# PetropoulakisPanagiotis/ICP-Variants

Measured on NVIDIA B200. Metric: icp_registrations_per_s, higher is better.
Workload: dtype f32

## Files before the change

### icp_variants_b200/csrc/clouds.cu

```cuda
#include "context.cuh"
#include <stdlib.h>

static int pick_T(int n, bool source = false) {
    if (!source) {
        int T = 3 * ICP_MAX_BITS_PER_AXIS;
        if (const char* e = getenv("ICP_GPU_TARGET_GRID_BITS")) { const int v = atoi(e); if (v >= 3 && v <= 3 * ICP_MAX_BITS_PER_AXIS) T = v; }
        return T;
    }
    int T = 3;
    while (T < 24 && (1ll << T) < (long long)ICP_SOURCE_CELLS_PER_POINT * (long long)(n > 0 ? n : 1)) ++T;
    if (T > 3 * ICP_MAX_BITS_PER_AXIS) T = 3 * ICP_MAX_BITS_PER_AXIS;
    return T;
}

static int ensure_sort(icp_gpu_ctx* ctx, icp_gpu_ctx::SortBufs& sb, int n, int T) {
    const size_t n1 = (size_t)(n > 0 ? n : 1);
    if (ensure(ctx, sb.keys_a, n1 * 4) || ensure(ctx, sb.keys_b, n1 * 4) || ensure(ctx, sb.idx_a, n1 * 4) || ensure(ctx, sb.idx_b, n1 * 4) ||
        ensure(ctx, sb.hist, icp_radix_hist_words(n, T) * 4) || ensure(ctx, sb.msd, ICP_MSD_WORDS * 4)) return ICP_GPU_E_CUDA;
    return 0;
}

static int upload_cloud(icp_gpu_ctx* ctx, const float* xyz, const float* nrm, const uint8_t* rgba, int64_t n, bool device_ptrs,
                        DeviceBuf& pts, DeviceBuf& nrmb, int kind ) {
    const size_t n1 = (size_t)(n > 0 ? n : 1);
    DeviceBuf& bbox = kind == 0 ? ctx->bbox : ctx->sbbox;
    DeviceBuf& grid = kind == 0 ? ctx->grid : ctx->sgrid;
    icp_gpu_ctx::SortBufs& sb = kind == 0 ? ctx->tsort : ctx->ssort;
    const int T = pick_T((int)n, kind == 1);
    if (kind == 0) ctx->T = T; else ctx->Ts = T;
    if (ensure(ctx, pts, n1 * sizeof(float4)) || ensure(ctx, nrmb, n1 * sizeof(float4)) || ensure(ctx, bbox, 64) || ensure(ctx, grid, sizeof(GridParams)) ||
        ensure_sort(ctx, sb, (int)n, T)) return ICP_GPU_E_CUDA;
    const long long hist_words = (long long)icp_radix_hist_words((int)n, T);
    if (n == 0) {
        CU(icp_launch_pack_cloud(nullptr, nullptr, nullptr, 0, (float4*)pts.p, (float4*)nrmb.p, (unsigned int*)bbox.p, T, (GridParams*)grid.p,
                                 (unsigned int*)sb.hist.p, hist_words, 1, ctx->stream));
        ctx->late_pending[kind] = false;
        return 0;
    }
    const float* dx = xyz; const float* dn = nrm; const uint8_t* dc = rgba;
    if (!device_ptrs) {
        DeviceBuf& stage = kind == 0 ? ctx->stage : ctx->stage2;
        const size_t sizes[] = {(size_t)n * 12, nrm ? (size_t)n * 12 : 0, rgba ? (size_t)n * 4 : 0};
        size_t off[3];
        if (ensure(ctx, stage, pack_segments(sizes, 3, off))) return ICP_GPU_E_CUDA;
        char* st = (char*)stage.p;
        if (ctx->packed_once[kind]) CU(cudaStreamWaitEvent(ctx->copy_stream, ctx->ev_packed[kind], 0));
        CU(cudaMemcpyAsync(st + off[0], xyz, sizes[0], cudaMemcpyHostToDevice, ctx->copy_stream));
        CU(cudaEventRecord(ctx->ev_xyz[kind], ctx->copy_stream));
        dx = (const float*)(st + off[0]);
        if (nrm) { CU(cudaMemcpyAsync(st + off[1], nrm, sizes[1], cudaMemcpyHostToDevice, ctx->copy_stream)); dn = (const float*)(st + off[1]); }
        if (rgba) { CU(cudaMemcpyAsync(st + off[2], rgba, sizes[2], cudaMemcpyHostToDevice, ctx->copy_stream)); dc = (const uint8_t*)(st + off[2]); }
        CU(cudaEventRecord(ctx->ev_copied[kind], ctx->copy_stream));
        CU(cudaStreamWaitEvent(ctx->stream, ctx->ev_xyz[kind], 0));
        ctx->late[kind].nrm = dn; ctx->late[kind].rgba = dc; ctx->late[kind].nrmo = (float4*)nrmb.p; ctx->late[kind].ready = ctx->ev_copied[kind];
    }
    ctx->late_pending[kind] = !device_ptrs;
    CU(icp_launch_pack_cloud(dx, dn, dc, (int)n, (float4*)pts.p, (float4*)nrmb.p, (unsigned int*)bbox.p, T, (GridParams*)grid.p,
                             (unsigned int*)sb.hist.p, hist_words, device_ptrs ? 1 : 0, ctx->stream));
    ctx->stats.n_kernel_launches += 1;
    return 0;
}

static int build_grid(icp_gpu_ctx* ctx) {
    const int n = ctx->n_tgt;
    const size_t n1 = (size_t)(n > 0 ? n : 1);
    if (ensure(ctx, ctx->tgt_pts_sorted, n1 * sizeof(float4)) || ensure(ctx, ctx->tgt_nrm_sorted, n1 * sizeof(float4)) ||
        ensure(ctx, ctx->lv_flags, n1 + 64) || ensure(ctx, ctx->lv_tiles, (n1 / 1024 + 2) * 4) ||
        ensure(ctx, ctx->delta_a, (n1 + 2) * 4) || ensure(ctx, ctx->delta_b, (n1 + 2) * 4) ||
        ensure(ctx, ctx->leaf_start, (n1 + 2) * 4) || ensure(ctx, ctx->leaf_rank, (n1 + 2) * 4) || ensure(ctx, ctx->bvh_desc, sizeof(BvhDesc)) ||
        ensure(ctx, ctx->bvh_box, icp_bvh_max_nodes(n) * 2 * sizeof(float4)) ||
        ensure(ctx, ctx->node_rank, (icp_bvh_max_nodes(n) + ICP_BVH_MAX_LEVELS) * 4) ||
        ensure(ctx, ctx->child_start, (icp_bvh_max_nodes(n) + ICP_BVH_MAX_LEVELS) * 4))
        return ICP_GPU_E_CUDA;
    ctx->adj_capacity = (int)(n1 / 4 + 64);
    ctx->adj1_capacity = (int)(n1 / 32 + 64);
    if (ensure(ctx, ctx->adj, (size_t)ctx->adj_capacity * 32 * 4) || ensure(ctx, ctx->adj_gap, (size_t)ctx->adj_capacity * 32 * 4) ||
        ensure(ctx, ctx->adj_box, (size_t)ctx->adj_capacity * 2 * sizeof(float4)) ||
        ensure(ctx, ctx->adj1, (size_t)ctx->adj1_capacity * 32 * 4) || ensure(ctx, ctx->adj1_box, (size_t)ctx->adj1_capacity * 2 * sizeof(float4)))
        return ICP_GPU_E_CUDA;
    int launches = 0;
    if (join_index(ctx)) return ICP_GPU_E_CUDA;
    CU(cudaEventRecord(ctx->ev[0], ctx->stream));
    CU(icp_launch_cloud_sort((const float4*)ctx->tgt_pts.p, (const float4*)ctx->tgt_nrm.p, n, ctx->T, (const GridParams*)ctx->grid.p,
                             (unsigned int*)ctx->tsort.keys_a.p, (unsigned int*)ctx->tsort.keys_b.p, (unsigned int*)ctx->tsort.idx_a.p,
                             (unsigned int*)ctx->tsort.idx_b.p, (unsigned int*)ctx->tsort.hist.p, (float4*)ctx->tgt_pts_sorted.p,
                             (float4*)ctx->tgt_nrm_sorted.p, (unsigned int*)ctx->tsort.msd.p, &ctx->tsort.keys_sorted, &ctx->tsort.msd_shift,
                             ctx->late_pending[0] ? &ctx->late[0] : nullptr, ctx->stream, &launches));
    if (ctx->late_pending[0]) { CU(cudaEventRecord(ctx->ev_packed[0], ctx->stream)); ctx->packed_once[0] = true; ctx->late_pending[0] = false; }
    cudaStream_t ts = getenv("ICP_GPU_NO_AUX_STREAM") ? ctx->stream : ctx->aux_stream;
    if (ts != ctx->stream) { CU(cudaEventRecord(ctx->ev_fork, ctx->stream)); CU(cudaStreamWaitEvent(ts, ctx->ev_fork, 0)); }
    CU(icp_launch_bvh_build((float4*)ctx->tgt_pts_sorted.p, (float4*)ctx->tgt_nrm_sorted.p, n, ctx->T, ctx->tsort.keys_sorted,
                            (const unsigned int*)ctx->bbox.p + 7, (unsigned char*)ctx->lv_flags.p, (unsigned int*)ctx->lv_tiles.p, (int*)ctx->delta_a.p,
                            (int*)ctx->delta_b.p, (unsigned int*)ctx->leaf_rank.p, (unsigned int*)ctx->leaf_start.p, (unsigned int*)ctx->node_rank.p,
                            (unsigned int*)ctx->child_start.p, (BvhDesc*)ctx->bvh_desc.p, (float4*)ctx->bvh_box.p, ctx->n_sms, ts, &launches));
    const bool bottom_up = !getenv("ICP_GPU_ADJ_FROM_ROOT");
    CU(icp_launch_leaf_adjacency((const BvhDesc*)ctx->bvh_desc.p, (const float4*)ctx->bvh_box.p, (const unsigned int*)ctx->child_start.p,
                                 (unsigned int*)ctx->adj1.p, (float4*)ctx->adj1_box.p, ctx->adj1_capacity, 1, nullptr, nullptr, nullptr, 0, ctx->n_sms, ts, &launches));
    CU(icp_launch_leaf_adjacency((const BvhDesc*)ctx->bvh_desc.p, (const float4*)ctx->bvh_box.p, (const unsigned int*)ctx->child_start.p,
                                 (unsigned int*)ctx->adj.p, (float4*)ctx->adj_box.p, ctx->adj_capacity, 0, (const unsigned int*)ctx->node_rank.p,
                                 bottom_up ? (const unsigned int*)ctx->adj1.p : nullptr, (const float4*)ctx->adj1_box.p, ctx->adj1_capacity, ctx->n_sms, ts, &launches,
                                 (float*)ctx->adj_gap.p));
    CU(cudaEventRecord(ctx->ev[1], ts));
    if (ts != ctx->stream) { CU(cudaEventRecord(ctx->ev_index_ready, ts)); ctx->index_pending = true; }
    ctx->stats.n_kernel_launches += (uint64_t)launches;
    ctx->grid_built = true;
    return 0;
}

static int build_source(icp_gpu_ctx* ctx) {
    const int n = ctx->n_src;
    const size_t n1 = (size_t)(n > 0 ? n : 1);
    if (ensure(ctx, ctx->src_pts, n1 * sizeof(float4)) || ensure(ctx, ctx->src_nrm, n1 * sizeof(float4))) return ICP_GPU_E_CUDA;
    int launches = 0;
    CU(icp_launch_cloud_sort((const float4*)ctx->src_raw_pts.p, (const float4*)ctx->src_raw_nrm.p, n, ctx->Ts, (const GridParams*)ctx->sgrid.p,
                             (unsigned int*)ctx->ssort.keys_a.p, (unsigned int*)ctx->ssort.keys_b.p, (unsigned int*)ctx->ssort.idx_a.p,
                             (unsigned int*)ctx->ssort.idx_b.p, (unsigned int*)ctx->ssort.hist.p, (float4*)ctx->src_pts.p,
                             (float4*)ctx->src_nrm.p, nullptr, &ctx->ssort.keys_sorted, &ctx->ssort.msd_shift,
                             ctx->late_pending[1] ? &ctx->late[1] : nullptr, ctx->stream, &launches));
    if (ctx->late_pending[1]) { CU(cudaEventRecord(ctx->ev_packed[1], ctx->stream)); ctx->packed_once[1] = true; ctx->late_pending[1] = false; }
    ctx->stats.n_kernel_launches += (uint64_t)launches;
    return 0;
}

int set_cloud(icp_gpu_ctx* ctx, bool target, const float* xyz, const float* nrm, const uint8_t* rgba, int64_t n, bool dev) {
    if (n < 0 || n > 0x7fffffff / 4 || (n > 0 && !xyz)) return fail(ctx, ICP_GPU_E_ARG, "bad cloud (n=%lld, xyz=%p)", (long long)n, (const void*)xyz);
    if (int rc = enter(ctx)) return rc;
    if (target) {
        if (join_index(ctx)) return ICP_GPU_E_CUDA;
        if (upload_cloud(ctx, xyz, nrm, rgba, n, dev, ctx->tgt_pts, ctx->tgt_nrm, 0)) return ICP_GPU_E_CUDA;
        ctx->n_tgt = (int)n;
        if (build_grid(ctx)) return ICP_GPU_E_CUDA;
    } else {
        if (upload_cloud(ctx, xyz, nrm, rgba, n, dev, ctx->src_raw_pts, ctx->src_raw_nrm, 1)) return ICP_GPU_E_CUDA;
        ctx->n_src = (int)n;
        ctx->src_finite_valid = false; ctx->src_rank_valid = false;
        const size_t n1 = (size_t)(n > 0 ? n : 1);
        if (ensure(ctx, ctx->match_pos, n1 * 4) || ensure(ctx, ctx->match_w, n1 * 4) || ensure(ctx, ctx->match_idx, n1 * 4) ||
            ensure(ctx, ctx->nn_pos, n1 * 4) || ensure(ctx, ctx->nn_leaf, n1 * 4) || ensure(ctx, ctx->qbuf, n1 * sizeof(float4)) ||
            ensure(ctx, ctx->seedbuf, n1 * sizeof(float4))) return ICP_GPU_E_CUDA;
        ctx->n_reduce_blocks = icp_reduce_blocks((int)n, ctx->n_sms);
        if (ensure(ctx, ctx->partials, (size_t)ctx->n_reduce_blocks * ICP_NRED * sizeof(double))) return ICP_GPU_E_CUDA;
        if (build_source(ctx)) return ICP_GPU_E_CUDA;
    }
    ctx->nn_stale = true;
    if (!dev && n > 0) CU(cudaEventSynchronize(ctx->ev_copied[target ? 0 : 1]));
    return ICP_GPU_OK;
}

int fetch_src_rank(icp_gpu_ctx* ctx) {
    if (ctx->src_rank_valid) return 0;
    const size_t n = (size_t)ctx->n_src;
    std::vector<int> order(n);
    if (n > 0) {
        if (ensure(ctx, ctx->order_dev, n * 4)) return ICP_GPU_E_CUDA;
        CU(icp_launch_extract_order((const float4*)ctx->src_pts.p, (int)n, (int*)ctx->order_dev.p, ctx->stream));
        CU(cudaMemcpyAsync(order.data(), ctx->order_dev.p, n * 4, cudaMemcpyDeviceToHost, ctx->stream));
        CU(cudaStreamSynchronize(ctx->stream));
    }
    ctx->src_rank.assign(n, 0);
    for (size_t p = 0; p < n; ++p) ctx->src_rank[(size_t)order[p]] = (int)p;
    ctx->src_rank_valid = true;
    return 0;
}

int fetch_src_finite(icp_gpu_ctx* ctx) {
    if (ctx->src_finite_valid) return 0;
    const size_t n = (size_t)ctx->n_src;
    std::vector<float4> p(n), m(n);
    CU(cudaMemcpyAsync(p.data(), ctx->src_raw_pts.p, n * sizeof(float4), cudaMemcpyDeviceToHost, ctx->stream));
    CU(cudaMemcpyAsync(m.data(), ctx->src_raw_nrm.p, n * sizeof(float4), cudaMemcpyDeviceToHost, ctx->stream));
    CU(cudaStreamSynchronize(ctx->stream));
    ctx->src_finite.resize(n);
    for (size_t i = 0; i < n; ++i) ctx->src_finite[i] = point_finite(&p[i].x, &m[i].x) ? 1 : 0;
    ctx->src_finite_valid = true;
    return 0;
}

int icp_gpu_set_target(icp_gpu_ctx* ctx, const float* xyz, const float* nrm, const uint8_t* rgba, int64_t n) { return set_cloud(ctx, true, xyz, nrm, rgba, n, false); }
int icp_gpu_set_source(icp_gpu_ctx* ctx, const float* xyz, const float* nrm, const uint8_t* rgba, int64_t n) { return set_cloud(ctx, false, xyz, nrm, rgba, n, false); }
int icp_gpu_set_target_dev(icp_gpu_ctx* ctx, const float* xyz, const float* nrm, const uint8_t* rgba, int64_t n) { return set_cloud(ctx, true, xyz, nrm, rgba, n, true); }
int icp_gpu_set_source_dev(icp_gpu_ctx* ctx, const float* xyz, const float* nrm, const uint8_t* rgba, int64_t n) { return set_cloud(ctx, false, xyz, nrm, rgba, n, true); }

int icp_gpu_cloud_from_depth(icp_gpu_ctx* ctx, const float* depth, const uint8_t* rgbx, const float K[9], const float E[16],
                             uint32_t width, uint32_t height, int keep_original_size, uint32_t downsample, float max_distance, int role,
                             float* xyz_out, float* nrm_out, uint8_t* rgba_out, int64_t* n_out) {
    if (!K) return ICP_GPU_E_ARG;
    if (!depth || width == 0 || height == 0 || downsample == 0 || (long long)width * height > 0x7fffffff / 4)
        return fail(ctx, ICP_GPU_E_ARG, "bad depth map (%p, %ux%u, downsample %u)", (const void*)depth, width, height, downsample);
    if (role < ICP_GPU_CLOUD_TARGET || role > ICP_GPU_CLOUD_ONLY) return fail(ctx, ICP_GPU_E_ARG, "role %d", role);
    if (int rc = enter(ctx)) return rc;
    const long long npx = (long long)width * height;
    DepthArgs a; memset(&a, 0, sizeof(a));
    a.width = width; a.height = height; a.downsample = downsample; a.keep_original_size = keep_original_size ? 1 : 0;
    a.n_candidates = (npx + downsample - 1) / downsample;
    a.fovX = K[0]; a.fovY = K[4]; a.cX = K[6]; a.cY = K[7];
    a.half_max_distance = max_distance / 2.f;
    for (int i = 0; i < 16; ++i) a.Einv[i] = (i % 5 == 0) ? 1.f : 0.f;
    if (E) {
        double m[4][8];
        for (int r = 0; r < 4; ++r) for (int c = 0; c < 4; ++c) { m[r][c] = E[r + 4 * c]; m[r][4 + c] = (r == c) ? 1.0 : 0.0; }
        for (int k = 0; k < 4; ++k) {
            int p = k; for (int i = k + 1; i < 4; ++i) if (fabs(m[i][k]) > fabs(m[p][k])) p = i;
            if (m[p][k] == 0.0) return fail(ctx, ICP_GPU_E_ARG, "singular depth extrinsics");
            if (p != k) for (int j = 0; j < 8; ++j) { const double t = m[k][j]; m[k][j] = m[p][j]; m[p][j] = t; }
            const double d = m[k][k];
            for (int j = 0; j < 8; ++j) m[k][j] /= d;
            for (int i = 0; i < 4; ++i) if (i != k) { const double f = m[i][k]; if (f != 0.0) for (int j = 0; j < 8; ++j) m[i][j] -= f * m[k][j]; }
        }
        for (int r = 0; r < 4; ++r) for (int c = 0; c < 4; ++c) a.Einv[r + 4 * c] = (float)m[r][4 + c];
    }
    const size_t nc = (size_t)a.n_candidates, nb = (nc + 255) / 256;
    const size_t depth_bytes = (size_t)npx * 4, color_bytes = rgbx ? (size_t)npx + 3 : 0;
    const size_t in_sizes[] = {depth_bytes, color_bytes}, sizes[] = {nc * 12, nc * 12, nc * 4, nc * 4, (nb + 2) * 4};
    size_t in_off[2], t[5];
    const size_t in_total = pack_segments(in_sizes, 2, in_off), t_end = pack_segments(sizes, 5, t);
    if (ensure(ctx, ctx->prep_in, in_total) || ensure(ctx, ctx->prep_tmp, t_end) || ensure(ctx, ctx->prep_out, t[3])) return ICP_GPU_E_CUDA;
    char* in = (char*)ctx->prep_in.p; char* tmp = (char*)ctx->prep_tmp.p; char* out = (char*)ctx->prep_out.p;
    CU(cudaMemcpyAsync(in, depth, depth_bytes, cudaMemcpyHostToDevice, ctx->stream));
    if (rgbx) CU(cudaMemcpyAsync(in + in_off[1], rgbx, color_bytes, cudaMemcpyHostToDevice, ctx->stream));
    int launches = 0;
    unsigned int* total = (unsigned int*)(tmp + t[4]) + nb;
    CU(icp_launch_depth_cloud((const float*)in, rgbx ? (const unsigned char*)(in + in_off[1]) : nullptr, a, (float*)tmp, (float*)(tmp + t[1]),
                              (unsigned char*)(tmp + t[2]), (unsigned int*)(tmp + t[3]), (unsigned int*)(tmp + t[4]), total,
                              (float*)out, (float*)(out + t[1]), (unsigned char*)(out + t[2]), ctx->stream, &launches));
    ctx->stats.n_kernel_launches += (uint64_t)launches;
    unsigned int n = 0;
    CU(cudaMemcpyAsync(&n, total, 4, cudaMemcpyDeviceToHost, ctx->stream));
    CU(cudaStreamSynchronize(ctx->stream));
    if (n_out) *n_out = (int64_t)n;
    if (n > 0) {
        if (xyz_out) CU(cudaMemcpyAsync(xyz_out, out, (size_t)n * 12, cudaMemcpyDeviceToHost, ctx->stream));
        if (nrm_out) CU(cudaMemcpyAsync(nrm_out, out + t[1], (size_t)n * 12, cudaMemcpyDeviceToHost, ctx->stream));
        if (rgba_out) CU(cudaMemcpyAsync(rgba_out, out + t[2], (size_t)n * 4, cudaMemcpyDeviceToHost, ctx->stream));
    }
    int rc = ICP_GPU_OK;
    if (role != ICP_GPU_CLOUD_ONLY)
        rc = set_cloud(ctx, role == ICP_GPU_CLOUD_TARGET, (const float*)out, (const float*)(out + t[1]), (const uint8_t*)(out + t[2]), (int64_t)n, true);
    if (xyz_out || nrm_out || rgba_out) CU(cudaStreamSynchronize(ctx->stream));
    return rc;
}

int icp_gpu_target_normals(icp_gpu_ctx* ctx, int32_t k, const float viewpoint[3], float* nrm_out, float* curvature_out) {
    if (k < 3 || k > 8) return fail(ctx, ICP_GPU_E_ARG, "k %d (3..8)", k);
    if (int rc = enter(ctx)) return rc;
    if (!ctx->grid_built) return fail(ctx, ICP_GPU_E_STATE, "no target cloud set");
    const int n = ctx->n_tgt;
    if (n <= 0) return ICP_GPU_OK;
    if (join_index(ctx)) return ICP_GPU_E_CUDA;
    if (ensure(ctx, ctx->nrm_out_dev, (size_t)n * 16 + 256)) return ICP_GPU_E_CUDA;
    NormalArgs a; memset(&a, 0, sizeof(a));
    a.pts = (const float4*)ctx->tgt_pts_sorted.p; a.n = n;
    a.bvh_box = (const float4*)ctx->bvh_box.p; a.bvh = (const BvhDesc*)ctx->bvh_desc.p; a.leaf_start = (const unsigned int*)ctx->leaf_start.p;
    a.leaf_rank = (const unsigned int*)ctx->leaf_rank.p; a.child_start = (const unsigned int*)ctx->child_start.p;
    a.adj = (const unsigned int*)ctx->adj.p; a.adj_box = (const float4*)ctx->adj_box.p; a.adj_capacity = ctx->adj_capacity;
    a.k = k;
    for (int i = 0; i < 3; ++i) a.vp[i] = viewpoint ? viewpoint[i] : 0.f;
    a.out_nrm = (float*)ctx->nrm_out_dev.p; a.out_curv = (float*)ctx->nrm_out_dev.p + 3 * (size_t)n;
    a.nrm_sorted = (float4*)ctx->tgt_nrm_sorted.p; a.nrm_orig = (float4*)ctx->tgt_nrm.p;
    CU(cudaMemsetAsync(ctx->nrm_out_dev.p, 0xFF, (size_t)n * 16, ctx->stream));
    CU(icp_launch_pca_normals(a, ctx->stream));
    ctx->stats.n_kernel_launches += 1;
    if (nrm_out) CU(cudaMemcpyAsync(nrm_out, a.out_nrm, (size_t)n * 12, cudaMemcpyDeviceToHost, ctx->stream));
    if (curvature_out) CU(cudaMemcpyAsync(curvature_out, a.out_curv, (size_t)n * 4, cudaMemcpyDeviceToHost, ctx->stream));
    if (nrm_out || curvature_out) CU(cudaStreamSynchronize(ctx->stream));
    return ICP_GPU_OK;
}
```

### icp_variants_b200/csrc/context.cu

```cuda
#include "context.cuh"
#include <stdarg.h>
#include <stdio.h>
#include <new>

int fail(icp_gpu_ctx* c, int code, const char* fmt, ...) {
    if (c) {
        va_list ap; va_start(ap, fmt);
        vsnprintf(c->err, sizeof(c->err), fmt, ap);
        va_end(ap);
    }
    return code;
}

int ensure(icp_gpu_ctx* ctx, DeviceBuf& b, size_t bytes, bool graph_reads) {
    if (bytes <= b.cap && b.p) return 0;
    if (graph_reads && ctx->graph_exec) { cudaGraphExecDestroy(ctx->graph_exec); ctx->graph_exec = nullptr; ctx->graph_key.clear(); }
    if (b.p) { cudaStreamSynchronize(ctx->stream); if (ctx->copy_stream) cudaStreamSynchronize(ctx->copy_stream); if (ctx->aux_stream) cudaStreamSynchronize(ctx->aux_stream); cudaFree(b.p); b.p = nullptr; b.cap = 0; }
    size_t want = bytes + bytes / 8 + 256;
    CU(cudaMalloc(&b.p, want));
    b.cap = want;
    return 0;
}

int enter(icp_gpu_ctx* ctx, bool idle) {
    if (!ctx) return ICP_GPU_E_ARG;
    if (idle && ctx->pending) return fail(ctx, ICP_GPU_E_STATE, "a registration is pending; call icp_gpu_estimate_pose_finish first");
    CU(cudaSetDevice(ctx->device));
    return 0;
}

int join_index(icp_gpu_ctx* ctx) {
    if (!ctx->index_pending) return 0;
    CU(cudaStreamWaitEvent(ctx->stream, ctx->ev_index_ready, 0));
    ctx->index_pending = false;
    return 0;
}

int upload_pose(icp_gpu_ctx* ctx, const float pose[16], float stop_rot, float stop_trans) {
    memcpy(ctx->h_pose, pose, 16 * sizeof(float));
    CU(cudaMemcpyAsync(ctx->pose_dev.p, ctx->h_pose, 16 * sizeof(float), cudaMemcpyHostToDevice, ctx->stream));
    CU(icp_launch_pose_init((DevState*)ctx->state.p, (const float*)ctx->pose_dev.p, ctx->stream, stop_rot, stop_trans));
    return 0;
}

int status_error(icp_gpu_ctx* ctx, int status, int iteration, const char* no_match) {
    if (status == 0) return ICP_GPU_OK;
    if (status == ICP_GPU_E_NO_MATCHES) return fail(ctx, status, no_match, iteration);
    if (status == ICP_GPU_E_PEER)
        return fail(ctx, status, "point-sharded registration: a peer's row did not arrive in time (iteration %d; rank %d of %d)", iteration, ctx->peer_rank, ctx->peer_world);
    if (iteration < 0) return fail(ctx, status, "singular / non-finite normal equations");
    return fail(ctx, status, "iteration %d: singular / non-finite normal equations", iteration);
}

size_t pack_segments(const size_t* sizes, int n, size_t* off) {
    size_t total = 0;
    for (int k = 0; k < n; ++k) { off[k] = total; total += (sizes[k] + 255) / 256 * 256; }
    return total;
}

int check_config(icp_gpu_ctx* ctx, const icp_gpu_config* c, const char* who) {
    if (c->metric < 0 || c->metric > 2) return fail(ctx, ICP_GPU_E_ARG, "%smetric %d", who, c->metric);
    if (c->minimizer < 0 || c->minimizer > 1) return fail(ctx, ICP_GPU_E_ARG, "%sminimizer %d", who, c->minimizer);
    if (c->matching < 0 || c->matching > 1) return fail(ctx, ICP_GPU_E_ARG, "%smatching %d", who, c->matching);
    if (c->selection < 0 || c->selection > 1) return fail(ctx, ICP_GPU_E_ARG, "%sselection %d", who, c->selection);
    if (c->selection_rng < 0 || c->selection_rng > 1) return fail(ctx, ICP_GPU_E_ARG, "%sselection_rng %d", who, c->selection_rng);
    if (c->weighting < 0 || c->weighting > 3) return fail(ctx, ICP_GPU_E_ARG, "%sweighting %d", who, c->weighting);
    if (c->nn_algorithm < 0 || c->nn_algorithm > 3) return fail(ctx, ICP_GPU_E_ARG, "%snn_algorithm %d", who, c->nn_algorithm);
    if (c->nn_algorithm == ICP_GPU_NN_BRUTE_NORM && c->color_icp) return fail(ctx, ICP_GPU_E_ARG, "%sthe norm-thresholded brute-force matcher is 3-D only (NearestNeighbor.h:63-69)", who);
    if (c->pyramid_mode != ICP_GPU_PYRAMID_STRIDE && c->pyramid_mode != ICP_GPU_PYRAMID_VOXEL) return fail(ctx, ICP_GPU_E_ARG, "%spyramid_mode %d", who, c->pyramid_mode);
    if (c->multires && c->pyramid_mode == ICP_GPU_PYRAMID_VOXEL && c->selection == ICP_GPU_SELECT_RANDOM && c->selection_rng == ICP_GPU_RNG_MT19937)
        return fail(ctx, ICP_GPU_E_ARG, "%svoxel pyramid levels are built on the device: use the device selection stream with them", who);
    if (c->n_iterations < 0 || c->n_iterations > ICP_MAX_ITERS) return fail(ctx, ICP_GPU_E_ARG, "%sn_iterations %d (max %d)", who, c->n_iterations, ICP_MAX_ITERS);
    if (c->lm_max_iterations < 0 || c->lm_max_iterations > 64) return fail(ctx, ICP_GPU_E_ARG, "%slm_max_iterations %d", who, c->lm_max_iterations);
    if (!(c->early_stop_rotation >= 0.f) || !(c->early_stop_translation >= 0.f)) return fail(ctx, ICP_GPU_E_ARG, "%searly-stop thresholds must be >= 0", who);
    if (!(c->weight_max_distance_sq >= 0.f)) return fail(ctx, ICP_GPU_E_ARG, "%sweight_max_distance_sq %g", who, (double)c->weight_max_distance_sq);
    if (c->matching == ICP_GPU_MATCH_PROJECTIVE && c->color_icp) return fail(ctx, ICP_GPU_E_ARG, "%scolour ICP is a k-NN variant (main.cpp:240-243)", who);
    return 0;
}

int icp_gpu_abi_version(void) { return ICP_GPU_ABI_VERSION; }

int icp_gpu_device_count(void) {
    int n = 0;
    if (cudaGetDeviceCount(&n) != cudaSuccess) { cudaGetLastError(); return 0; }
    return n;
}

void icp_gpu_default_config(icp_gpu_config* cfg) {
    if (!cfg) return;
    memset(cfg, 0, sizeof(*cfg));
    cfg->metric = ICP_GPU_METRIC_P2P; cfg->minimizer = ICP_GPU_MIN_LINEAR; cfg->matching = ICP_GPU_MATCH_KNN;
    cfg->selection = ICP_GPU_SELECT_ALL; cfg->proba = 1.0; cfg->seed = 0; cfg->selection_rng = ICP_GPU_RNG_MT19937;
    cfg->weighting = ICP_GPU_WEIGHT_CONSTANT; cfg->rejection = 1; cfg->max_distance_sq = 0.0003f;
    cfg->color_icp = 0; cfg->multires = 0; cfg->pyramid_mode = ICP_GPU_PYRAMID_STRIDE; cfg->n_iterations = 20;
    cfg->lm_max_iterations = 10; cfg->nn_algorithm = ICP_GPU_NN_AUTO; cfg->use_graph = 1; cfg->collect_stats = 1;
    cfg->weight_max_distance_sq = 0.0f; cfg->early_stop_rotation = 0.0f; cfg->early_stop_translation = 0.0f;
}

int icp_gpu_create(icp_gpu_ctx** out, int device) {
    if (!out) return ICP_GPU_E_ARG;
    *out = nullptr;
    int n = 0;
    if (cudaGetDeviceCount(&n) != cudaSuccess || n <= 0) { cudaGetLastError(); return ICP_GPU_E_CUDA; }
    if (device < 0 || device >= n) return ICP_GPU_E_ARG;
    icp_gpu_ctx* ctx = new (std::nothrow) icp_gpu_ctx();
    if (!ctx) return ICP_GPU_E_CUDA;
    ctx->err[0] = 0; ctx->device = device;
    memset(&ctx->stats, 0, sizeof(ctx->stats));
    icp_gpu_default_config(&ctx->cfg);
    cudaDeviceProp prop;
    bool ok = cudaSetDevice(device) == cudaSuccess && cudaGetDeviceProperties(&prop, device) == cudaSuccess;
    if (ok && prop.major < 10) ok = false;
    if (ok) ctx->n_sms = prop.multiProcessorCount;
    ok = ok && cudaStreamCreateWithFlags(&ctx->own_stream, cudaStreamNonBlocking) == cudaSuccess;
    ctx->stream = ctx->own_stream;
    ok = ok && cudaStreamCreateWithFlags(&ctx->copy_stream, cudaStreamNonBlocking) == cudaSuccess;
    ok = ok && cudaStreamCreateWithFlags(&ctx->aux_stream, cudaStreamNonBlocking) == cudaSuccess;
    ok = ok && cudaEventCreateWithFlags(&ctx->ev_fork, cudaEventDisableTiming) == cudaSuccess && cudaEventCreateWithFlags(&ctx->ev_index_ready, cudaEventDisableTiming) == cudaSuccess;
    for (int c = 0; c < ICP_MAX_MATCH_CHUNKS - 1; ++c)
        ok = ok && cudaStreamCreateWithFlags(&ctx->chunks.stream[c], cudaStreamNonBlocking) == cudaSuccess &&
             cudaEventCreateWithFlags(&ctx->chunks.done[c], cudaEventDisableTiming) == cudaSuccess;
    ok = ok && cudaEventCreateWithFlags(&ctx->chunks.fork, cudaEventDisableTiming) == cudaSuccess;
    for (int i = 0; ok && i < 4; ++i) ok = cudaEventCreate(&ctx->ev[i]) == cudaSuccess;
    for (int i = 0; ok && i < 2; ++i) ok = cudaEventCreateWithFlags(&ctx->ev_xyz[i], cudaEventDisableTiming) == cudaSuccess && cudaEventCreateWithFlags(&ctx->ev_copied[i], cudaEventDisableTiming) == cudaSuccess &&
                                           cudaEventCreateWithFlags(&ctx->ev_packed[i], cudaEventDisableTiming) == cudaSuccess;
    ok = ok && cudaMallocHost((void**)&ctx->h_pose, 16 * sizeof(float)) == cudaSuccess;
    ok = ok && cudaMallocHost((void**)&ctx->h_history, 16 * sizeof(float) * ICP_MAX_ITERS) == cudaSuccess;
    ok = ok && cudaMallocHost((void**)&ctx->h_state, sizeof(DevState)) == cudaSuccess;
    ok = ok && cudaMallocHost((void**)&ctx->h_desc, sizeof(IterDesc) * DESC_TOTAL) == cudaSuccess;
    ok = ok && ensure(ctx, ctx->state, sizeof(DevState)) == 0 && ensure(ctx, ctx->desc, sizeof(IterDesc) * DESC_TOTAL) == 0 &&
         ensure(ctx, ctx->pose_dev, 64) == 0 && ensure(ctx, ctx->history, 16 * sizeof(float) * ICP_MAX_ITERS) == 0 &&
         ensure(ctx, ctx->mask, 256) == 0;
    if (ok) ok = cudaMemsetAsync(ctx->state.p, 0, sizeof(DevState), ctx->stream) == cudaSuccess && cudaStreamSynchronize(ctx->stream) == cudaSuccess;
    if (!ok) { cudaGetLastError(); icp_gpu_destroy(ctx); return ICP_GPU_E_CUDA; }
    *out = ctx;
    return ICP_GPU_OK;
}

int icp_gpu_destroy(icp_gpu_ctx* ctx) {
    if (!ctx) return ICP_GPU_OK;
    cudaSetDevice(ctx->device);
    if (ctx->stream) cudaStreamSynchronize(ctx->stream);
    if (ctx->copy_stream) cudaStreamSynchronize(ctx->copy_stream);
    if (ctx->aux_stream) cudaStreamSynchronize(ctx->aux_stream);
    if (ctx->graph_exec) cudaGraphExecDestroy(ctx->graph_exec);
    peer_close(ctx);
    if (ctx->peer_box) cudaFree(ctx->peer_box);
    if (ctx->h_pose) cudaFreeHost(ctx->h_pose);
    if (ctx->h_history) cudaFreeHost(ctx->h_history);
    if (ctx->h_state) cudaFreeHost(ctx->h_state);
    if (ctx->h_desc) cudaFreeHost(ctx->h_desc);
    for (int i = 0; i < 4; ++i) if (ctx->ev[i]) cudaEventDestroy(ctx->ev[i]);
    for (int i = 0; i < 2; ++i) { if (ctx->ev_xyz[i]) cudaEventDestroy(ctx->ev_xyz[i]); if (ctx->ev_copied[i]) cudaEventDestroy(ctx->ev_copied[i]); if (ctx->ev_packed[i]) cudaEventDestroy(ctx->ev_packed[i]); }
    if (ctx->ev_fork) cudaEventDestroy(ctx->ev_fork);
    for (int c = 0; c < ICP_MAX_MATCH_CHUNKS - 1; ++c)
        if (ctx->chunks.stream[c]) { cudaStreamSynchronize(ctx->chunks.stream[c]); cudaStreamDestroy(ctx->chunks.stream[c]); }
    for (int c = 0; c < ICP_MAX_MATCH_CHUNKS - 1; ++c) if (ctx->chunks.done[c]) cudaEventDestroy(ctx->chunks.done[c]);
    if (ctx->chunks.fork) cudaEventDestroy(ctx->chunks.fork);
    if (ctx->ev_index_ready) cudaEventDestroy(ctx->ev_index_ready);
    if (ctx->aux_stream) cudaStreamDestroy(ctx->aux_stream);
    if (ctx->copy_stream) cudaStreamDestroy(ctx->copy_stream);
    if (ctx->own_stream) cudaStreamDestroy(ctx->own_stream);
    delete ctx;
    return ICP_GPU_OK;
}

const char* icp_gpu_last_error(const icp_gpu_ctx* ctx) { return ctx ? ctx->err : "null context"; }

int icp_gpu_set_stream(icp_gpu_ctx* ctx, void* cuda_stream) {
    if (int rc = enter(ctx)) return rc;
    CU(cudaStreamSynchronize(ctx->stream));
    CU(cudaStreamSynchronize(ctx->aux_stream));
    ctx->index_pending = false;
    ctx->stream = cuda_stream ? (cudaStream_t)cuda_stream : ctx->own_stream;
    return ICP_GPU_OK;
}

int icp_gpu_synchronize(icp_gpu_ctx* ctx) {
    if (int rc = enter(ctx, false)) return rc;
    if (join_index(ctx)) return ICP_GPU_E_CUDA;
    CU(cudaStreamSynchronize(ctx->stream));
    return ICP_GPU_OK;
}

int icp_gpu_set_config(icp_gpu_ctx* ctx, const icp_gpu_config* c) {
    if (!ctx || !c) return ICP_GPU_E_ARG;
    if (int rc = check_config(ctx, c, "")) return rc;
    ctx->cfg = *c;
    return ICP_GPU_OK;
}

int icp_gpu_get_config(const icp_gpu_ctx* ctx, icp_gpu_config* c) {
    if (!ctx || !c) return ICP_GPU_E_ARG;
    *c = ctx->cfg;
    return ICP_GPU_OK;
}

int icp_gpu_set_camera(icp_gpu_ctx* ctx, const float K[9], uint32_t width, uint32_t height) {
    if (!ctx || !K) return ICP_GPU_E_ARG;
    memcpy(ctx->K, K, 9 * sizeof(float));
    ctx->width = width; ctx->height = height; ctx->have_camera = true;
    return ICP_GPU_OK;
}

int icp_gpu_get_stats(icp_gpu_ctx* ctx, icp_gpu_stats* out) {
    if (!ctx || !out) return ICP_GPU_E_ARG;
    *out = ctx->stats;
    return ICP_GPU_OK;
}

int icp_gpu_measure_fp32_peak(icp_gpu_ctx* ctx, int32_t mode, double* tflops_out) {
    if (!tflops_out || mode < 0 || mode > 1) return ICP_GPU_E_ARG;
    if (int rc = enter(ctx)) return rc;
    CU(icp_measure_fp32_peak(mode, ctx->n_sms, ctx->stream, tflops_out));
    return ICP_GPU_OK;
}
```

### icp_variants_b200/csrc/context.cuh

```cuda
#pragma once
#include "icp_internal.cuh"
#include <string.h>
#include <vector>

#define DESC_QUERY (ICP_MAX_ITERS)
#define DESC_TOTAL (ICP_MAX_ITERS + 1)

struct DeviceBuf {
    void* p = nullptr; size_t cap = 0;
    DeviceBuf() = default;
    DeviceBuf(DeviceBuf&& o) noexcept : p(o.p), cap(o.cap) { o.p = nullptr; o.cap = 0; }
    ~DeviceBuf() { if (p) cudaFree(p); }
};

struct icp_gpu_ctx {
    int device = 0, n_sms = 148;
    cudaStream_t own_stream = nullptr, stream = nullptr;
    cudaStream_t copy_stream = nullptr;
    cudaStream_t aux_stream = nullptr;
    cudaEvent_t ev_fork = nullptr, ev_index_ready = nullptr;
    MatchChunks chunks;
    bool index_pending = false;
    cudaEvent_t ev_copied[2] = {nullptr, nullptr};
    cudaEvent_t ev_xyz[2] = {nullptr, nullptr};
    IcpLatePack late[2]; bool late_pending[2] = {false, false};
    cudaEvent_t ev_packed[2] = {nullptr, nullptr};
    bool packed_once[2] = {false, false};
    DeviceBuf stage2;
    icp_gpu_config cfg;
    float K[9]; uint32_t width = 0, height = 0; bool have_camera = false;
    DeviceBuf stage, src_raw_pts, src_raw_nrm, src_pts, src_nrm, tgt_pts, tgt_nrm, tgt_pts_sorted, tgt_nrm_sorted;
    int n_src = -1, n_tgt = -1;
    std::vector<uint8_t> src_finite;
    bool src_finite_valid = false;
    std::vector<int> src_rank;
    bool src_rank_valid = false;
    DeviceBuf grid, bbox, bvh_box, bvh_desc, leaf_start, leaf_rank, node_rank, child_start, adj, adj_box, adj1, adj1_box, adj_gap;
    struct SortBufs { DeviceBuf keys_a, keys_b, idx_a, idx_b, hist, msd; unsigned int* keys_sorted = nullptr; int msd_shift = 0; };
    SortBufs tsort, ssort;
    DeviceBuf lv_flags, lv_tiles, delta_a, delta_b;
    int adj1_capacity = 0;
    int adj_capacity = 0;
    int T = 0; bool grid_built = false; double index_ms = 0.0;
    bool nn_stale = true;
    DeviceBuf sgrid, sbbox, order_dev, voxel_table;
    int Ts = 0;
    DeviceBuf state, desc, mask, match_pos, match_w, match_idx, nn_pos, nn_leaf, qbuf, seedbuf, partials, pose_dev, history;
    DeviceBuf nrm_out_dev;
    DeviceBuf prep_in, prep_tmp, prep_out, gt_src, gt_ref, met_partial, met_out;
    DeviceBuf scratch[16];
    DeviceBuf batch_io, batch_scratch, batch_plan;
    long long n_gt = 0; int last_iters = 0;
    float* h_pose = nullptr; float* h_history = nullptr; DevState* h_state = nullptr;
    IterDesc* h_desc = nullptr;
    int n_reduce_blocks = 1;
    cudaGraphExec_t graph_exec = nullptr;
    std::vector<long long> graph_key;
    uint64_t graph_launches = 0;
    bool pending = false; int pending_iters = 0;
    bool shard_open = false; int shard_algo = 0, shard_iters = 0;
    void* peer_box = nullptr;
    void* peer_ptr[ICP_MAX_PEERS] = {nullptr};
    bool peer_ipc[ICP_MAX_PEERS] = {false};
    int peer_world = 0, peer_rank = 0, peer_plan_check = 0;
    uint64_t peer_epoch = 0;
    icp_gpu_stats stats;
    cudaEvent_t ev[4] = {nullptr, nullptr, nullptr, nullptr};
    char err[512];
};

int fail(icp_gpu_ctx* c, int code, const char* fmt, ...);

#define CU(call)                                                                                         \
    do {                                                                                                 \
        cudaError_t e__ = (call);                                                                        \
        if (e__ != cudaSuccess) return fail(ctx, ICP_GPU_E_CUDA, "%s: %s", #call, cudaGetErrorString(e__)); \
    } while (0)

int ensure(icp_gpu_ctx* ctx, DeviceBuf& b, size_t bytes, bool graph_reads = true);
int enter(icp_gpu_ctx* ctx, bool idle = true);
int join_index(icp_gpu_ctx* ctx);
int upload_pose(icp_gpu_ctx* ctx, const float pose[16], float stop_rot = 0.f, float stop_trans = 0.f);
int status_error(icp_gpu_ctx* ctx, int status, int iteration, const char* no_match);
size_t pack_segments(const size_t* sizes, int n, size_t* off);

inline size_t mask_words(long long n) { return ((size_t)(n > 0 ? n : 1) + 31) / 32; }

inline IterDesc all_points_desc() {
    IterDesc d; memset(&d, 0, sizeof(d));
    d.stride = 1; d.mask_word_offset = -1; d.proba = -1.0f;
    return d;
}

inline bool point_finite(const float* p, const float* m) {
    return isfinite(p[0]) && isfinite(p[1]) && isfinite(p[2]) && (!m || (isfinite(m[0]) && isfinite(m[1]) && isfinite(m[2])));
}

int check_config(icp_gpu_ctx* ctx, const icp_gpu_config* c, const char* who);
int set_cloud(icp_gpu_ctx* ctx, bool target, const float* xyz, const float* nrm, const uint8_t* rgba, int64_t n, bool dev);
int fetch_src_rank(icp_gpu_ctx* ctx);
int fetch_src_finite(icp_gpu_ctx* ctx);
void draw_selection_masks(const icp_gpu_config& cfg, const IcpSchedule& sch, long long n, const uint8_t* finite, uint32_t* out);
int choose_algorithm(const icp_gpu_ctx* c);
int check_ready(icp_gpu_ctx* ctx);
void fill_match_args(icp_gpu_ctx* c, MatchArgs& a, int algo, int desc_index, bool want_idx);
void fill_reduce_args(icp_gpu_ctx* c, ReduceArgs& r, int algo, int solve);
int refresh_seeds(icp_gpu_ctx* ctx, int algo, bool allow_seed);
void peer_close(icp_gpu_ctx* ctx);
```

### icp_variants_b200/csrc/icp_internal.cuh

```cuda
#pragma once
#include <cuda_runtime.h>
#include <stdint.h>
#include <math.h>
#include "../../include/icp_gpu.h"

#define ICP_MAX_ITERS 256
#define ICP_NRED 32
#define ICP_REDUCE_THREADS 256
#define ICP_MAX_PEERS 8
#define ICP_MATCH_THREADS 128
#define ICP_LEAF_MAX 8
#define ICP_CELLS_PER_POINT 32
#define ICP_SOURCE_CELLS_PER_POINT 4
#define ICP_MAX_BITS_PER_AXIS 10

__device__ __forceinline__ float pmul(float a, float b) { return __fmul_rn(a, b); }
__device__ __forceinline__ float padd(float a, float b) { return __fadd_rn(a, b); }
__device__ __forceinline__ float psub(float a, float b) { return __fsub_rn(a, b); }
__device__ __forceinline__ float pdiv(float a, float b) { return __fdiv_rn(a, b); }
__device__ __forceinline__ bool finite3(float x, float y, float z) { return isfinite(x) && isfinite(y) && isfinite(z); }

struct GridParams {
    float o[3];
    float h[3];
    float inv_h[3];
    float delta[3];
    int bits[3];
    int T;
    unsigned long long axis_seq;
    int n_finite;
    int pad;
    unsigned char bitpos[3][ICP_MAX_BITS_PER_AXIS];
    unsigned char pad2[2];
};

#define ICP_BVH_MAX_LEVELS 7
struct BvhDesc {
    int n_levels;
    int n_leaves;
    int count[ICP_BVH_MAX_LEVELS];
    int offset[ICP_BVH_MAX_LEVELS];
    int coffset[ICP_BVH_MAX_LEVELS];
};

struct IterDesc {
    int stride;
    int filter_finite;
    int mask_word_offset;
    unsigned int rng_key;
    float proba;
    int pad0, pad1, pad2;
};

struct IcpSchedule {
    int coarsest;
    int levels;
    int n_iters;
};
__host__ __device__ inline IcpSchedule icp_schedule(int n_iterations, int multires, long long n) {
    IcpSchedule s; s.coarsest = 1; s.levels = 1; s.n_iters = n_iterations;
    if (!multires) return s;
    float res = 1.0f; int sz = (int)n;
    for (;;) { sz = (int)(sz / 2.0); if (sz < 100) break; res *= 2.0f; }
    s.coarsest = (int)res;
    for (int c = s.coarsest; c > 1; c /= 2) ++s.levels;
    if (s.levels > s.n_iters) s.n_iters = s.levels;
    return s;
}
__host__ __device__ inline int icp_schedule_stride(const IcpSchedule& s, int i) { return i < s.levels ? s.coarsest >> i : 1; }
__host__ __device__ inline int icp_schedule_level(const IcpSchedule& s, int i) { return i < s.levels ? i : s.levels - 1; }

struct LmState {
    double x[6], cand[6], cost, H[36], g[6], scale[6], diag[6];
    double radius, decrease, model_change;
    int iter, done, reuse_diag, invalid, step_ok, have_cand;
};

struct DevState {
    float pose[16];
    float nrm[9];
    int iter;
    int iters_done;
    int status;
    unsigned int ticket;
    unsigned int ticket2;
    float mean_s[3];
    float mean_d[3];
    double mean_s64[3], mean_d64[3];
    unsigned long long n_queries, n_matched, n_evals, n_nodes;
    LmState lm;
    double shard_partials[ICP_NRED];
    unsigned int xchg_seq;
    int pad_xchg;
    float stop_rot, stop_trans; int converged; int pad_stop;
    unsigned long long prof[6];
};

struct PeerBox {
    double row[2][ICP_MAX_PEERS][ICP_NRED];
    unsigned int flag[2][ICP_MAX_PEERS];
};

struct PeerXchg {
    int world, rank;
    unsigned long long timeout_ns;
    int plan_check;
    int pad_;
    PeerBox* box[ICP_MAX_PEERS];
};

struct MatchArgs {
    const float4* src_pts;
    const float4* src_nrm;
    int n_src;
    const unsigned int* mask;
    const IterDesc* desc;
    const DevState* state_ro;
    DevState* state;
    const float4* tgt_pts;
    const float4* tgt_nrm;
    int n_tgt;
    const float4* bvh_box;
    const BvhDesc* bvh;
    const unsigned int* leaf_start;
    const unsigned int* child_start;
    const unsigned int* leaf_rank;
    const unsigned int* adj; const float4* adj_box; int adj_capacity;
    const float* adj_gap;
    const unsigned int* adj1; const float4* adj1_box; int adj1_capacity; const unsigned int* node_rank;
    int* nn_leaf;
    float fx, fy, cx, cy; unsigned int width, height;
    int weighting, rejection, color_icp;
    float max_d2;
    float weight_max_d2;
    int* match_pos;
    float* match_w;
    int* match_idx;
    int* nn_pos;
    float4* seedbuf;
    float4* qbuf;
    int desc_index;
    int use_seed;
    int brute_norm;
    int proj_tiled;
    int fast_path;
    int collect_stats;
    int skip_finish;
    int q_begin, q_end;
    int group_min;
};

#define ICP_MAX_MATCH_CHUNKS 8
struct MatchChunks {
    int n = 1;
    cudaStream_t stream[ICP_MAX_MATCH_CHUNKS - 1] = {};
    cudaEvent_t done[ICP_MAX_MATCH_CHUNKS - 1] = {};
    cudaEvent_t fork = nullptr;
};

struct ReduceArgs {
    const float4* src_pts; const float4* src_nrm; int n_src;
    DevState* state;
    const float4* tgt_pts; const float4* tgt_nrm;
    const int* match_pos; const float* match_w;
    double* partials;
    float* pose_history;
    int metric; int solve;
    int fused; const int* nn_pos; int n_tgt; const unsigned int* mask; const IterDesc* desc; int desc_index;
    int weighting, rejection; float max_d2, weight_max_d2;
    int profile;
    PeerXchg peer;
};

#define ICP_BATCH_MAX_TARGET ICP_GPU_BATCH_MAX_TARGET
#define ICP_BATCH_THREADS 512
#define ICP_BATCH_LM_THREADS 256
struct BatchCfg {
    int n_iterations, multires, weighting, rejection, lm_max_iterations;
    int mt_mask;
    float max_d2, weight_max_d2;
    float proba;
    unsigned int seed;
    float stop_rot, stop_trans;
};
struct BatchArgs {
    const float* src_xyz; const float* src_nrm; const long long* src_off;
    const float* tgt_xyz; const float* tgt_nrm; const long long* tgt_off;
    const float* poses_in;
    float* poses_out; int* n_iter_out; int* status_out;
    float* history;
    int history_rows;
    int2* scratch;
    const BatchCfg* cfgs; const int* cfg_index;
    const int* pairs;
    const unsigned int* mask; const long long* mask_off;
};
cudaError_t icp_launch_batch(const BatchArgs& a, int metric, int lm, int n_pairs, int max_tgt, cudaStream_t s);

cudaError_t icp_launch_transform(const float* in, long long n, const float pose16[16], int normals, float* out, cudaStream_t s);
cudaError_t icp_launch_apply_weights(int method, float max_d2, const float* sp, const float* sn, const unsigned int* sc, const float* tp, const float* tn,
                                     const unsigned int* tc, long long n_tgt, const int* idx, float* w, long long n, cudaStream_t s);
cudaError_t icp_launch_pack_pairs(const float* s, const float* sn, const float* t, const float* tn, const float* w, int n, float4* sp4, float4* sn4,
                                  float4* tp4, float4* tn4, int* pos, float* wo, cudaStream_t st);
cudaError_t icp_measure_fp32_peak(int mode, int n_sms, cudaStream_t s, double* tflops);
cudaError_t icp_launch_pack_cloud(const float* xyz, const float* nrm, const uint8_t* rgba, int n, float4* pts, float4* nrmo,
                                  unsigned int* scratch, int T, GridParams* grid, unsigned int* hist, long long hist_words, int with_normals, cudaStream_t s);
struct IcpLatePack { const float* nrm; const uint8_t* rgba; float4* nrmo; cudaEvent_t ready; };
struct IcpRadixPlan { int n_pass; int shift[4]; int bits[4]; int ipt; int tile_items; int n_tiles; int tiles_pad; };
void icp_radix_plan(int n, int T, IcpRadixPlan* p);
size_t icp_radix_hist_words(int n, int T);
#define ICP_MSD_WORDS 257
cudaError_t icp_launch_cloud_sort(const float4* pts_in, const float4* nrm_in, int n, int T, const GridParams* grid,
                                  unsigned int* keys_a, unsigned int* keys_b, unsigned int* idx_a, unsigned int* idx_b,
                                  unsigned int* hist, float4* pts_sorted, float4* nrm_sorted, unsigned int* msd_start,
                                  unsigned int** keys_sorted_out, int* msd_shift_out, const IcpLatePack* late, cudaStream_t s, int* n_launches);
size_t icp_bvh_max_nodes(int n);
cudaError_t icp_launch_bvh_build(float4* pts_sorted, float4* nrm_sorted, int n, int T, const unsigned int* keys,
                                 const unsigned int* nonfinite, unsigned char* flags, unsigned int* tile_count,
                                 int* delta_a, int* delta_b, unsigned int* leaf_rank, unsigned int* leaf_start, unsigned int* node_rank,
                                 unsigned int* child_start, BvhDesc* bvh_dev, float4* box, int n_sms, cudaStream_t s, int* n_launches);
cudaError_t icp_launch_voxel_level(const float4* pts_sorted, const float4* nrm_sorted, int n, const GridParams* grid, int T, int D,
                                   unsigned int* table, unsigned int* mask, size_t mask_words, cudaStream_t s, int* n_launches);
cudaError_t icp_launch_leaf_adjacency(const BvhDesc* bvh_dev, const float4* box, const unsigned int* child_start, unsigned int* adj,
                                      float4* adj_box, int capacity, int level, const unsigned int* node_rank, const unsigned int* adj1,
                                      const float4* adj1_box, int adj1_capacity, int n_sms, cudaStream_t s, int* n_launches,
                                      float* adj_gap = nullptr);
cudaError_t icp_launch_extract_order(const float4* pts_sorted, int n, int* order, cudaStream_t s);
cudaError_t icp_launch_fill_int(int* p, int n, int v, cudaStream_t s);
cudaError_t icp_launch_seed_from_keys(const float4* src_pts, int n_src, const DevState* st, const GridParams* grid, const unsigned int* keys, int n_tgt,
                                      const unsigned int* nonfinite, const unsigned int* msd_start, int msd_shift, const unsigned int* leaf_rank,
                                      int* nn_pos, int* nn_leaf, int reset, cudaStream_t s);
struct DepthArgs {
    unsigned int width, height, downsample; int keep_original_size;
    long long n_candidates;
    float fovX, fovY, cX, cY, half_max_distance;
    float Einv[16];
};
cudaError_t icp_launch_depth_cloud(const float* depth, const unsigned char* color, const DepthArgs& a, float* pts_tmp, float* nrm_tmp,
                                   unsigned char* rgba_tmp, unsigned int* flag, unsigned int* block_count, unsigned int* total,
                                   float* pts_out, float* nrm_out, unsigned char* rgba_out, cudaStream_t s, int* n_launches);
cudaError_t icp_launch_gt_from_source(const float4* src_raw, long long n, const float* pose16_dev, float* gt_src, float* gt_ref, cudaStream_t s);
int icp_metrics_blocks(long long m, int n_sms);
cudaError_t icp_launch_metrics(const float* src, const float* ref, long long m, const float* history, int n_iters, int n_blocks, double* partial,
                               float* rmse, float* centroid, double* bench, cudaStream_t s, int* n_launches);
struct NormalArgs {
    const float4* pts; int n;
    const float4* bvh_box; const BvhDesc* bvh; const unsigned int* leaf_start; const unsigned int* leaf_rank; const unsigned int* child_start;
    const unsigned int* adj; const float4* adj_box; int adj_capacity;
    int k; float vp[3];
    float* out_nrm; float* out_curv;
    float4* nrm_sorted; float4* nrm_orig;
};
cudaError_t icp_launch_pca_normals(const NormalArgs& a, cudaStream_t s);
cudaError_t icp_launch_match(const MatchArgs& a, int algorithm, int n_sms, cudaStream_t s, int* n_launches, cudaEvent_t after_prep = nullptr,
                             const MatchChunks* chunks = nullptr);
cudaError_t icp_launch_pose_init(DevState* st, const float* pose_dev16, cudaStream_t s, float stop_rot = 0.f, float stop_trans = 0.f);
cudaError_t icp_launch_reduce(const ReduceArgs& a, int n_blocks, cudaStream_t s, int* n_launches);
cudaError_t icp_launch_reduce_phase(const ReduceArgs& a, int n_blocks, int phase, cudaStream_t s, int* n_launches);
int icp_reduce_blocks(int n_src, int n_sms);
cudaError_t icp_launch_shard_apply(DevState* st, int mode, float* history, cudaStream_t s);
cudaError_t icp_launch_lm(const ReduceArgs& a, int n_blocks, int lm_max_iterations, cudaStream_t s, int* n_launches);

__device__ __forceinline__ void mat4_mul_pinned(const float* A, const float* B, float* C) {
    float T[16];
#pragma unroll
    for (int j = 0; j < 4; ++j)
#pragma unroll
        for (int i = 0; i < 4; ++i)
            T[i + 4 * j] = padd(padd(padd(pmul(A[i], B[4 * j]), pmul(A[i + 4], B[1 + 4 * j])), pmul(A[i + 8], B[2 + 4 * j])),
                                pmul(A[i + 12], B[3 + 4 * j]));
#pragma unroll
    for (int k = 0; k < 16; ++k) C[k] = T[k];
}

__device__ __forceinline__ void inv_transpose3_pinned(const float* P, float* N) {
    const float r00 = P[0], r10 = P[1], r20 = P[2], r01 = P[4], r11 = P[5], r21 = P[6], r02 = P[8], r12 = P[9], r22 = P[10];
    const float c00 = psub(pmul(r11, r22), pmul(r12, r21)), c01 = psub(pmul(r12, r20), pmul(r10, r22)), c02 = psub(pmul(r10, r21), pmul(r11, r20));
    const float c10 = psub(pmul(r02, r21), pmul(r01, r22)), c11 = psub(pmul(r00, r22), pmul(r02, r20)), c12 = psub(pmul(r01, r20), pmul(r00, r21));
    const float c20 = psub(pmul(r01, r12), pmul(r02, r11)), c21 = psub(pmul(r02, r10), pmul(r00, r12)), c22 = psub(pmul(r00, r11), pmul(r01, r10));
    const float det = padd(padd(pmul(r00, c00), pmul(r01, c01)), pmul(r02, c02));
    const float id = pdiv(1.0f, det);
    N[0] = pmul(c00, id); N[1] = pmul(c01, id); N[2] = pmul(c02, id);
    N[3] = pmul(c10, id); N[4] = pmul(c11, id); N[5] = pmul(c12, id);
    N[6] = pmul(c20, id); N[7] = pmul(c21, id); N[8] = pmul(c22, id);
}

__device__ __forceinline__ void xform_point(const float* P, float x, float y, float z, float& ox, float& oy, float& oz) {
    ox = padd(padd(padd(pmul(P[0], x), pmul(P[4], y)), pmul(P[8], z)), P[12]);
    oy = padd(padd(padd(pmul(P[1], x), pmul(P[5], y)), pmul(P[9], z)), P[13]);
    oz = padd(padd(padd(pmul(P[2], x), pmul(P[6], y)), pmul(P[10], z)), P[14]);
}
__device__ __forceinline__ void xform_normal(const float* N, float x, float y, float z, float& ox, float& oy, float& oz) {
    ox = padd(padd(pmul(N[0], x), pmul(N[1], y)), pmul(N[2], z));
    oy = padd(padd(pmul(N[3], x), pmul(N[4], y)), pmul(N[5], z));
    oz = padd(padd(pmul(N[6], x), pmul(N[7], y)), pmul(N[8], z));
}

__device__ __forceinline__ float unit_hash(unsigned int key, unsigned int k) {
    unsigned int x = k * 0x9E3779B9u + key;
    x ^= x >> 16; x *= 0x7FEB352Du; x ^= x >> 15; x *= 0x846CA68Bu; x ^= x >> 16;
    x += key * 0x85EBCA6Bu; x ^= x >> 16; x *= 0x7FEB352Du; x ^= x >> 15; x *= 0x846CA68Bu; x ^= x >> 16;
    return (float)(x >> 8) * (1.0f / 16777216.0f);
}

__device__ __forceinline__ bool query_active(const IterDesc& d, const unsigned int* __restrict__ mask, const float4& p4, const float4& n4) {
    const unsigned int orig = (unsigned int)__float_as_int(p4.w);
    if (d.stride > 1 && (orig % (unsigned int)d.stride) != 0u) return false;
    if (d.filter_finite && !(finite3(p4.x, p4.y, p4.z) && finite3(n4.x, n4.y, n4.z))) return false;
    if (d.mask_word_offset >= 0 && !((__ldg(&mask[d.mask_word_offset + (orig >> 5)]) >> (orig & 31u)) & 1u)) return false;
    if (d.proba >= 0.0f && !(unit_hash(d.rng_key, orig) < d.proba)) return false;
    return true;
}

__device__ __forceinline__ bool match_weight_and_reject(int weighting, int rejection, float max_d2, float sx, float sy, float sz,
                                                        float snx, float sny, float snz, unsigned int s_rgba, const float4 tp,
                                                        const float4 tn, float& w) {
    if (weighting != ICP_GPU_WEIGHT_CONSTANT) {
        w = 0.0f;
        if (weighting == ICP_GPU_WEIGHT_DISTANCES || weighting == ICP_GPU_WEIGHT_COLORS) {
            if (finite3(sx, sy, sz) && finite3(tp.x, tp.y, tp.z)) {
                const float d0 = psub(sx, tp.x), d1 = psub(sy, tp.y), d2 = psub(sz, tp.z);
                const float q = pdiv(padd(padd(pmul(d0, d0), pmul(d1, d1)), pmul(d2, d2)), max_d2);
                w = (float)(1.0 - (double)q);
            }
        }
        if (weighting == ICP_GPU_WEIGHT_NORMALS) {
            if (finite3(snx, sny, snz) && finite3(tn.x, tn.y, tn.z))
                w = padd(padd(pmul(snx, tn.x), pmul(sny, tn.y)), pmul(snz, tn.z));
        }
        if (weighting == ICP_GPU_WEIGHT_COLORS) {
            const unsigned int t_rgba = __float_as_uint(tn.w);
            int s = 0;
#pragma unroll
            for (int k = 0; k < 3; ++k) {
                const int e = (int)((((s_rgba >> (8 * k)) & 0xFFu) - ((t_rgba >> (8 * k)) & 0xFFu)) & 0xFFu);
                s += e * e;
            }
            const float cw = (float)(1.0 - (double)pdiv((float)s, 195075.0f));
            w = pmul(w, cw);
        }
    }
    if (rejection == 1) {
        const float dot = padd(padd(pmul(snx, tn.x), pmul(sny, tn.y)), pmul(snz, tn.z));
        const float na = __fsqrt_rn(padd(padd(pmul(snx, snx), pmul(sny, sny)), pmul(snz, snz)));
        const float nb = __fsqrt_rn(padd(padd(pmul(tn.x, tn.x), pmul(tn.y, tn.y)), pmul(tn.z, tn.z)));
        const float c = pdiv(dot, pmul(na, nb));
        if (c <= 0.5f && c >= -1.0f) return false;
    }
    return true;
}

template <int H>
__device__ __forceinline__ void halve_step(double (&v)[32], int lane) {
    const bool upper = (lane & H) != 0;
#pragma unroll
    for (int k = 0; k < H; ++k) {
        const double send = upper ? v[k] : v[k + H];
        const double keep = upper ? v[k + H] : v[k];
        v[k] = keep + __shfl_xor_sync(0xFFFFFFFFu, send, H);
    }
}
__device__ __forceinline__ void warp_reduce_scatter32(double (&v)[32], int lane) {
    halve_step<16>(v, lane); halve_step<8>(v, lane); halve_step<4>(v, lane); halve_step<2>(v, lane); halve_step<1>(v, lane);
}

static __device__ int solve6_dev(double* A , double* b, double* x) {
    for (int k = 0; k < 6; ++k) {
        int p = k; double mx = fabs(A[k * 6 + k]);
        for (int i = k + 1; i < 6; ++i) if (fabs(A[i * 6 + k]) > mx) { mx = fabs(A[i * 6 + k]); p = i; }
        if (!(mx > 0.0)) return -1;
        if (p != k) {
            for (int j = 0; j < 6; ++j) { const double t = A[k * 6 + j]; A[k * 6 + j] = A[p * 6 + j]; A[p * 6 + j] = t; }
            const double t = b[k]; b[k] = b[p]; b[p] = t;
        }
        for (int i = k + 1; i < 6; ++i) {
            const double f = A[i * 6 + k] / A[k * 6 + k];
            for (int j = k; j < 6; ++j) A[i * 6 + j] -= f * A[k * 6 + j];
            b[i] -= f * b[k];
        }
    }
    for (int i = 5; i >= 0; --i) {
        double s = b[i];
        for (int j = i + 1; j < 6; ++j) s -= A[i * 6 + j] * x[j];
        x[i] = s / A[i * 6 + i];
    }
    for (int i = 0; i < 6; ++i) if (!isfinite(x[i])) return -1;
    return 0;
}


__device__ __forceinline__ void mat4_identity_dev(float* M) {
    for (int i = 0; i < 16; ++i) M[i] = (i % 5 == 0) ? 1.f : 0.f;
}


__device__ __forceinline__ bool increment_is_small(const float* inc, float stop_rot, float stop_trans) {
    if (!(stop_rot > 0.f) || !(stop_trans > 0.f)) return false;
    double f = 0.0;
    for (int c = 0; c < 3; ++c) for (int r = 0; r < 3; ++r) { const double d = (double)inc[r + 4 * c] - (r == c ? 1.0 : 0.0); f += d * d; }
    const double theta = 2.0 * asin(fmin(sqrt(f) / (2.0 * sqrt(2.0)), 1.0));
    const double t = sqrt((double)inc[12] * inc[12] + (double)inc[13] * inc[13] + (double)inc[14] * inc[14]);
    return theta <= (double)stop_rot && t <= (double)stop_trans;
}

static __device__ void apply_increment(DevState* st, const float* inc, int rc, float* history) {
    if (st->status == 0) {
        if (rc != 0) st->status = rc;
        else {
            float np[16];
            mat4_mul_pinned(inc, st->pose, np);
            for (int i = 0; i < 16; ++i) st->pose[i] = np[i];
            inv_transpose3_pinned(st->pose, st->nrm);
            if (history) for (int i = 0; i < 16; ++i) history[16 * st->iters_done + i] = np[i];
            st->iters_done += 1;
            if (increment_is_small(inc, st->stop_rot, st->stop_trans)) st->converged = 1;
        }
    }
    st->iter += 1;
}


__device__ __forceinline__ void st_release_sys_u32(unsigned int* p, unsigned int v) {
    asm volatile("st.release.sys.global.u32 [%0], %1;" ::"l"(p), "r"(v) : "memory");
}
__device__ __forceinline__ unsigned int ld_acquire_sys_u32(const unsigned int* p) {
    unsigned int v;
    asm volatile("ld.acquire.sys.global.u32 %0, [%1];" : "=r"(v) : "l"(p) : "memory");
    return v;
}
__device__ __forceinline__ double ld_relaxed_sys_f64(const double* p) {
    double v;
    asm volatile("ld.relaxed.sys.global.f64 %0, [%1];" : "=d"(v) : "l"(p) : "memory");
    return v;
}
__device__ __forceinline__ unsigned long long global_timer_ns() {
    unsigned long long t;
    asm volatile("mov.u64 %0, %%globaltimer;" : "=l"(t));
    return t;
}

#define ICP_PEER_POISON 0xFFFFFFFFu
template <int THREADS>
__device__ __forceinline__ void peer_exchange_row(const PeerXchg& px, DevState* st, double (*red)[32], double (*fin)[32]) {
    static_assert(THREADS / 32 >= ICP_MAX_PEERS, "one warp per peer");
    const int lane = threadIdx.x & 31, w = threadIdx.x >> 5;
    __shared__ int s_failed;
    if (threadIdx.x == 0) s_failed = (*reinterpret_cast<volatile int*>(&st->status) == ICP_GPU_E_PEER) ? 1 : 0;
    __syncthreads();
    const bool failed_before = s_failed != 0;
    const unsigned int seq = st->xchg_seq + 1u;
    const int slot = (int)(seq & 1u);
    bool lost = false;
    if (!failed_before && w < px.world) {
        if (w != px.rank) {
            PeerBox* theirs = px.box[w];
            theirs->row[slot][px.rank][lane] = lane == 31 ? (double)px.plan_check : fin[0][lane];
            __threadfence_system();
            __syncwarp();
            if (lane == 0) st_release_sys_u32(&theirs->flag[slot][px.rank], seq);
            const PeerBox* mine = px.box[px.rank];
            const unsigned long long t0 = global_timer_ns();
            for (;;) {
                const unsigned int f = ld_acquire_sys_u32(&mine->flag[slot][w]);
                if (f == seq) break;
                if (f == ICP_PEER_POISON || global_timer_ns() - t0 > px.timeout_ns) { lost = true; break; }
                __nanosleep(64);
            }
            red[w][lane] = ld_relaxed_sys_f64(&mine->row[slot][w][lane]);
        } else {
            red[w][lane] = lane == 31 ? (double)px.plan_check : fin[0][lane];
        }
    }
    if (!failed_before && !lost && w < px.world && lane == 31 && red[w][31] != (double)px.plan_check) lost = true;
    if (lost && (lane == 0 || lane == 31)) { atomicCAS(&st->status, 0, ICP_GPU_E_PEER); s_failed = 1; }
    __syncthreads();
    if (s_failed) {
        if (w < px.world && w != px.rank && lane < 2) st_release_sys_u32(&px.box[w]->flag[lane][px.rank], ICP_PEER_POISON);
        if (failed_before) return;
    }
    if (threadIdx.x < 32) {
        double s = 0.0;
        for (int j = 0; j < px.world; ++j) s += red[j][threadIdx.x];
        fin[0][threadIdx.x] = s;
    }
    if (threadIdx.x == 0) st->xchg_seq = seq;
    __syncthreads();
}

template <int THREADS>
__device__ __forceinline__ bool grid_reduce_row(double (&v)[32], double* __restrict__ partials, unsigned int* ticket,
                                                double (*red)[32], double (*fin)[32], bool* is_last,
                                                const PeerXchg* px = nullptr, DevState* px_state = nullptr) {
    const int lane = threadIdx.x & 31, wid = threadIdx.x >> 5;
    warp_reduce_scatter32(v, lane);
    red[wid][lane] = v[0];
    __syncthreads();
    if (threadIdx.x < 32) {
        double s = 0.0;
#pragma unroll
        for (int w = 0; w < THREADS / 32; ++w) s += red[w][threadIdx.x];
        partials[(size_t)blockIdx.x * ICP_NRED + threadIdx.x] = s;
        __threadfence();
    }
    __syncthreads();
    if (threadIdx.x == 0) {
        const unsigned int t = atomicAdd(ticket, 1u);
        *is_last = (t == gridDim.x - 1);
    }
    __syncthreads();
    if (!*is_last) return false;
    __threadfence();
    {
        const int c = threadIdx.x & 31, g = threadIdx.x >> 5;
        double s0 = 0.0, s1 = 0.0, s2 = 0.0, s3 = 0.0, s4 = 0.0, s5 = 0.0, s6 = 0.0, s7 = 0.0;
        const int step = THREADS / 32, nb = (int)gridDim.x;
        int b = g;
        for (; b + 7 * step < nb; b += 8 * step) {
            const double x0 = __ldcg(&partials[(size_t)b * ICP_NRED + c]);
            const double x1 = __ldcg(&partials[(size_t)(b + step) * ICP_NRED + c]);
            const double x2 = __ldcg(&partials[(size_t)(b + 2 * step) * ICP_NRED + c]);
            const double x3 = __ldcg(&partials[(size_t)(b + 3 * step) * ICP_NRED + c]);
            const double x4 = __ldcg(&partials[(size_t)(b + 4 * step) * ICP_NRED + c]);
            const double x5 = __ldcg(&partials[(size_t)(b + 5 * step) * ICP_NRED + c]);
            const double x6 = __ldcg(&partials[(size_t)(b + 6 * step) * ICP_NRED + c]);
            const double x7 = __ldcg(&partials[(size_t)(b + 7 * step) * ICP_NRED + c]);
            s0 += x0; s1 += x1; s2 += x2; s3 += x3; s4 += x4; s5 += x5; s6 += x6; s7 += x7;
        }
        for (; b < nb; b += step) s0 += __ldcg(&partials[(size_t)b * ICP_NRED + c]);
        fin[g][c] = ((s0 + s1) + (s2 + s3)) + ((s4 + s5) + (s6 + s7));
    }
    __syncthreads();
    if (threadIdx.x < 32) {
        double s = 0.0;
#pragma unroll
        for (int g = 0; g < THREADS / 32; ++g) s += fin[g][threadIdx.x];
        fin[0][threadIdx.x] = s;
    }
    __syncthreads();
    if (threadIdx.x == 0) *ticket = 0;
    if (px && px->world > 1) peer_exchange_row<THREADS>(*px, px_state, red, fin);
    return true;
}
```

### icp_variants_b200/csrc/match.cu

```cuda
#include "icp_internal.cuh"
#include <limits.h>

#define MINF_F (-INFINITY)
#define FLT_BIG 3.4028234e38f

struct Query {
    float x, y, z;
    float cr, cg, cb;
};

struct Best { float d; int idx; int pos; };

__device__ __forceinline__ bool better(float d, int idx, const Best& b) { return d < b.d || (d == b.d && idx < b.idx); }

__device__ __forceinline__ bool better_key(float d, int idx, const Best& b) {
    return (((unsigned long long)__float_as_uint(d) << 32) | (unsigned int)idx) <
           (((unsigned long long)__float_as_uint(b.d) << 32) | (unsigned int)b.idx);
}
__device__ __forceinline__ void best_init(Best& b, float max_d2) {
    if (max_d2 < 0.f) { b.d = 0.f; b.idx = 0; }
    else { b.d = fminf(max_d2, FLT_BIG); b.idx = INT_MAX; }
    b.pos = -1;
}

__device__ __forceinline__ float color_feature(unsigned int rgba, int k) {
    return pmul(1.0f / 255.0f, (float)((rgba >> (8 * k)) & 0xFFu));
}

__device__ __forceinline__ float dist3(const Query& q, const float4 c) {
    const float dx = psub(q.x, c.x), dy = psub(q.y, c.y), dz = psub(q.z, c.z);
    return padd(padd(pmul(dx, dx), pmul(dy, dy)), pmul(dz, dz));
}
__device__ __forceinline__ float dist6_tail(const Query& q, float d, unsigned int rgba) {
    const float dr = psub(q.cr, color_feature(rgba, 0)), dg = psub(q.cg, color_feature(rgba, 1)), db = psub(q.cb, color_feature(rgba, 2));
    d = padd(d, pmul(dr, dr)); d = padd(d, pmul(dg, dg)); d = padd(d, pmul(db, db));
    return d;
}

template <bool COLOR>
__device__ __forceinline__ float dist2(const Query& q, const float4 c, float best, const float4* __restrict__ nrm, unsigned int i) {
    float d = dist3(q, c);
    if (COLOR) {
        if (d > best) return d;
        d = dist6_tail(q, d, __float_as_uint(__ldg(&nrm[i].w)));
    }
    return d;
}

__device__ __forceinline__ unsigned int x86_float_to_u32(float t) {
    if (!(fabsf(t) < 9223372036854775808.0f)) return 0u;
    return (unsigned int)(long long)t;
}

struct PoseSm { float P[16]; float N[9]; };

__device__ __forceinline__ void load_pose(PoseSm& sm, const DevState* st) {
    if (threadIdx.x < 16) sm.P[threadIdx.x] = st->pose[threadIdx.x];
    else if (threadIdx.x < 25) sm.N[threadIdx.x - 16] = st->nrm[threadIdx.x - 16];
    __syncthreads();
}

__device__ __forceinline__ void finish_match(const MatchArgs& a, int p, bool matched, float w_const, int t_idx, int t_pos,
                                             float sx, float sy, float sz, float snx, float sny, float snz, unsigned int s_rgba,
                                             unsigned int& n_matched) {
    int out_idx = -1, out_pos = -1; float w = 0.0f;
    if (matched) {
        const float4 tn = __ldg(&a.tgt_nrm[t_pos]);
        float4 tp = make_float4(0.f, 0.f, 0.f, 0.f);
        if (a.weighting != ICP_GPU_WEIGHT_CONSTANT) tp = __ldg(&a.tgt_pts[t_pos]);
        w = w_const;
        if (match_weight_and_reject(a.weighting, a.rejection, a.weight_max_d2, sx, sy, sz, snx, sny, snz, s_rgba, tp, tn, w)) {
            out_idx = t_idx; out_pos = t_pos; ++n_matched;
        }
    }
    a.match_pos[p] = out_pos;
    a.match_w[p] = w;
    if (a.match_idx) a.match_idx[p] = out_idx;
}

__device__ __forceinline__ void write_no_query(const MatchArgs& a, int p) {
    a.match_pos[p] = -1; a.match_w[p] = 0.0f; if (a.match_idx) a.match_idx[p] = -1;
}

__device__ __forceinline__ void flush_stats(const MatchArgs& a, unsigned int nq, unsigned int nm, unsigned int ev, unsigned int nd) {
    if (!a.collect_stats) return;
    DevState* st = a.state;
    nq = __reduce_add_sync(0xFFFFFFFFu, nq); nm = __reduce_add_sync(0xFFFFFFFFu, nm);
    ev = __reduce_add_sync(0xFFFFFFFFu, ev); nd = __reduce_add_sync(0xFFFFFFFFu, nd);
    if ((threadIdx.x & 31) == 0) {
        if (nq) atomicAdd(&st->n_queries, (unsigned long long)nq);
        if (nm) atomicAdd(&st->n_matched, (unsigned long long)nm);
        if (ev) atomicAdd(&st->n_evals, (unsigned long long)ev);
        if (nd) atomicAdd(&st->n_nodes, (unsigned long long)nd);
    }
}

__device__ __forceinline__ bool prepare_query(const MatchArgs& a, const IterDesc& d, const PoseSm& sm, int p, Query& q,
                                              float& snx, float& sny, float& snz, unsigned int& s_rgba) {
    const float4 p4 = __ldg(&a.src_pts[p]);
    const float4 n4 = __ldg(&a.src_nrm[p]);
    if (!query_active(d, a.mask, p4, n4)) return false;
    xform_point(sm.P, p4.x, p4.y, p4.z, q.x, q.y, q.z);
    xform_normal(sm.N, n4.x, n4.y, n4.z, snx, sny, snz);
    s_rgba = __float_as_uint(n4.w);
    q.cr = color_feature(s_rgba, 0); q.cg = color_feature(s_rgba, 1); q.cb = color_feature(s_rgba, 2);
    return true;
}

#ifdef ICP_TIMELINE
#define ICP_TL_ITER 12
#define ICP_TL_WARPS 40960
__device__ unsigned long long g_timeline[2][2][ICP_TL_WARPS][2];
__device__ __forceinline__ unsigned long long tl_now() { unsigned long long t; asm volatile("mov.u64 %0, %%globaltimer;" : "=l"(t)); return t; }
extern "C" int icp_gpu_debug_timeline(unsigned long long* out, int reset) {
    if (reset) { void* p = nullptr; cudaGetSymbolAddress(&p, g_timeline); return (int)cudaMemset(p, 0, sizeof(g_timeline)); }
    return (int)cudaMemcpyFromSymbol(out, g_timeline, sizeof(g_timeline));
}
#define TL_BEGIN(k, it, chunk) const int tl_w = (int)((blockIdx.x * blockDim.x + threadIdx.x) >> 5), tl_c = (chunk); \
    const bool tl_on = (it) == ICP_TL_ITER && (threadIdx.x & 31) == 0 && tl_w < ICP_TL_WARPS; if (tl_on) g_timeline[k][tl_c][tl_w][0] = tl_now()
#define TL_END(k) if (tl_on) g_timeline[k][tl_c][tl_w][1] = tl_now()
#else
#define TL_BEGIN(k, it, chunk)
#define TL_END(k)
#endif

#ifndef BVH_WARPS
#define BVH_WARPS 4
#endif
#define BVH_STACK (32 * ICP_BVH_MAX_LEVELS)

__device__ __forceinline__ float box_dist2(const Query& q, const float4 lo, const float4 hi) {
    const float gx = fmaxf(fmaxf(psub(lo.x, q.x), psub(q.x, hi.x)), 0.0f);
    const float gy = fmaxf(fmaxf(psub(lo.y, q.y), psub(q.y, hi.y)), 0.0f);
    const float gz = fmaxf(fmaxf(psub(lo.z, q.z), psub(q.z, hi.z)), 0.0f);
    return padd(padd(pmul(gx, gx), pmul(gy, gy)), pmul(gz, gz));
}

template <bool COLOR>
__device__ __forceinline__ float box_dist2c(const Query& q, const float4 lo, const float4 hi) {
    float d = box_dist2(q, lo, hi);
    if (COLOR) {
        const unsigned int cl = __float_as_uint(lo.w), ch = __float_as_uint(hi.w);
        const float gr = fmaxf(fmaxf(psub(color_feature(cl, 0), q.cr), psub(q.cr, color_feature(ch, 0))), 0.0f);
        const float gg = fmaxf(fmaxf(psub(color_feature(cl, 1), q.cg), psub(q.cg, color_feature(ch, 1))), 0.0f);
        const float gb = fmaxf(fmaxf(psub(color_feature(cl, 2), q.cb), psub(q.cb, color_feature(ch, 2))), 0.0f);
        d = padd(d, pmul(gr, gr)); d = padd(d, pmul(gg, gg)); d = padd(d, pmul(gb, gb));
    }
    return d;
}

template <bool COLOR>
__device__ __forceinline__ void bvh_scan_leaves(const MatchArgs& a, const Query& q, Best& b, float& bound, unsigned int ls, unsigned int le,
                                                float clb, bool keep, int lane, unsigned int& ev, unsigned int& nd) {
    const unsigned int FULL = 0xFFFFFFFFu;
    unsigned int key = keep ? __float_as_uint(clb) : 0xFFFFFFFFu;
    for (;;) {
        const unsigned int kmin = __reduce_min_sync(FULL, key);
        if (kmin == 0xFFFFFFFFu || __uint_as_float(kmin) > bound) break;
        const int src = __ffs((int)__ballot_sync(FULL, key == kmin)) - 1;
        const unsigned int s0 = __shfl_sync(FULL, ls, src), e0 = __shfl_sync(FULL, le, src);
        if (lane == src) key = 0xFFFFFFFFu;
        const unsigned int i = s0 + lane;
        if (i < e0) {
            const float4 pt = __ldg(&a.tgt_pts[i]);
            const float dd = dist2<COLOR>(q, pt, b.d, a.tgt_nrm, i);
            const int idx = __float_as_int(pt.w);
            if (better_key(dd, idx, b)) { b.d = dd; b.idx = idx; b.pos = (int)i; }
            ++ev;
        }
        if (lane == 0) ++nd;
        bound = __uint_as_float(__reduce_min_sync(FULL, __float_as_uint(b.d)));
    }
}

template <bool COLOR>
__device__ __forceinline__ void bvh_visit(const MatchArgs& a, const BvhDesc& bvh, const Query& q, Best& b, float& bound, int L,
                                          unsigned int first, unsigned int last, unsigned int* st_node, float* st_lb, int& top, int lane,
                                          unsigned int lt_mask, unsigned int& ev, unsigned int& nd) {
    const unsigned int FULL = 0xFFFFFFFFu;
    const unsigned int c = first + lane;
    float clb = FLT_BIG; bool keep = false;
    unsigned int ls = 0u, le = 0u;
    if (c < last) {
        const float4 lo = __ldg(&a.bvh_box[2 * (size_t)(bvh.offset[L] + c)]), hi = __ldg(&a.bvh_box[2 * (size_t)(bvh.offset[L] + c) + 1]);
        if (L == 0) { ls = __ldg(&a.leaf_start[c]); le = __ldg(&a.leaf_start[c + 1]); }
        clb = box_dist2c<COLOR>(q, lo, hi);
        keep = !(clb > bound);
    }
    if (L == 0) { bvh_scan_leaves<COLOR>(a, q, b, bound, ls, le, clb, keep, lane, ev, nd); return; }
    const unsigned int mk = __ballot_sync(FULL, keep);
    if (keep) { const int s = top + __popc(mk & lt_mask); st_node[s] = ((unsigned int)L << 27) | c; st_lb[s] = clb; }
    top += __popc(mk);
    __syncwarp();
}

template <bool COLOR>
__device__ __forceinline__ void thread_scan_range(const MatchArgs& a, const Query& q, Best& b, int& bleaf, unsigned int leaf, unsigned int ls, unsigned int le, unsigned int& ev) {
    if (b.d < 0.f) return;
    float run = __uint_as_float(__float_as_uint(b.d) + 1u);
    int pos = -1;
    for (unsigned int i = ls; i < le; ++i) {
        const float4 pt = __ldg(&a.tgt_pts[i]);
        const float dd = dist2<COLOR>(q, pt, run, a.tgt_nrm, i);
        if (dd < run) { run = dd; pos = (int)i; }
    }
    ev += le - ls;
    if (pos >= 0) {
        const int idx = __float_as_int(__ldg(&a.tgt_pts[pos].w));
        if (better_key(run, idx, b)) { b.d = run; b.idx = idx; b.pos = pos; bleaf = (int)leaf; }
    }
}
template <bool COLOR>
__device__ __forceinline__ void thread_scan_leaf(const MatchArgs& a, const Query& q, Best& b, int& bleaf, unsigned int leaf, unsigned int& ev) {
    thread_scan_range<COLOR>(a, q, b, bleaf, leaf, __ldg(&a.leaf_start[leaf]), __ldg(&a.leaf_start[leaf + 1]), ev);
}

#ifndef PREP_THREADS
#define PREP_THREADS 256
#endif
#ifndef PREP_MIN_BLOCKS
#define PREP_MIN_BLOCKS 5
#endif
template <bool COLOR, bool STATS>
__global__ void __launch_bounds__(PREP_THREADS, PREP_MIN_BLOCKS * 256 / PREP_THREADS) knn_prep_kernel(const MatchArgs a) {
    __shared__ PoseSm sm;
    const int p = a.q_begin + blockIdx.x * blockDim.x + threadIdx.x;
    float4 p4 = make_float4(0.f, 0.f, 0.f, 0.f), n4 = p4;
    int sp_raw = -1, leaf_raw = -1;
    if (p < a.q_end) {
        p4 = __ldg(&a.src_pts[p]); n4 = __ldg(&a.src_nrm[p]);
        sp_raw = a.nn_pos[p]; leaf_raw = a.nn_leaf[p];
    }
    if (a.desc_index < 0 && a.state_ro->converged) return;
    const int desc_i = a.desc_index >= 0 ? a.desc_index : a.state_ro->iter;
    TL_BEGIN(0, a.state_ro->iter, a.q_begin > 0 ? 1 : 0);
    load_pose(sm, a.state_ro);
    const IterDesc d = a.desc[desc_i];
    unsigned int ev = 0, nd = 0;
    if (p < a.q_end) {
        float4 o = make_float4(__int_as_float(0x7fc00000), 0.f, 0.f, n4.w);
        float4 seed = make_float4(0.f, 0.f, 0.f, __int_as_float(-2));
        if (query_active(d, a.mask, p4, n4)) {
            float x, y, z;
            xform_point(sm.P, p4.x, p4.y, p4.z, x, y, z);
            if (finite3(x, y, z)) {
                o.x = x; o.y = y; o.z = z;
                const int sp = (a.fast_path && a.use_seed) ? sp_raw : -1;
                const int seed_leaf = (sp >= 0 && sp < a.n_tgt) ? leaf_raw : -1;
                if (seed_leaf >= 0 && seed_leaf < a.adj_capacity) {
                    Query q; q.x = x; q.y = y; q.z = z;
                    const unsigned int s_rgba = __float_as_uint(n4.w);
                    q.cr = color_feature(s_rgba, 0); q.cg = color_feature(s_rgba, 1); q.cb = color_feature(s_rgba, 2);
                    Best b; best_init(b, a.max_d2);
                    int bleaf = -1;
                    thread_scan_leaf<COLOR>(a, q, b, bleaf, (unsigned int)seed_leaf, ev); ++nd;
                    seed = make_float4(b.d, __int_as_float(b.idx), __int_as_float(b.pos), __int_as_float(-1));
                    if (b.d < FLT_BIG) {
                        const float r = __fmul_ru(__fsqrt_ru(b.d), 1.00001f);
                        const float4 ilo = __ldg(&a.adj_box[2 * (size_t)seed_leaf]), ihi = __ldg(&a.adj_box[2 * (size_t)seed_leaf + 1]);
                        const bool inside = __fsub_rd(x, r) >= ilo.x && __fadd_ru(x, r) <= ihi.x && __fsub_rd(y, r) >= ilo.y &&
                                            __fadd_ru(y, r) <= ihi.y && __fsub_rd(z, r) >= ilo.z && __fadd_ru(z, r) <= ihi.z;
                        if (inside) {
                            const int na = __float_as_int(ilo.w);
                            const unsigned int* list = a.adj + (size_t)seed_leaf * 32;
                            unsigned int todo = 0;
                            const float* gap = a.adj_gap ? a.adj_gap + (size_t)seed_leaf * 32 : nullptr;
                            const float lim = (gap && bleaf == seed_leaf) ? __fmul_ru(__fmul_ru(4.0f, b.d), 1.00001f) : FLT_BIG;
                            for (int j = 0; j < na; ++j) {
                                if (gap && __ldg(&gap[j]) > lim) break;
                                const unsigned int leaf = __ldg(&list[j]);
                                const float clb = box_dist2c<COLOR>(q, __ldg(&a.bvh_box[2 * (size_t)leaf]), __ldg(&a.bvh_box[2 * (size_t)leaf + 1]));
                                if (!(clb > b.d)) todo |= 1u << j;
                            }
                            while (todo) {
                                const int j = __ffs((int)todo) - 1; todo &= todo - 1u;
                                const unsigned int leaf = __ldg(&list[j]);
                                const float clb = box_dist2c<COLOR>(q, __ldg(&a.bvh_box[2 * (size_t)leaf]), __ldg(&a.bvh_box[2 * (size_t)leaf + 1]));
                                if (!(clb > b.d)) { thread_scan_leaf<COLOR>(a, q, b, bleaf, leaf, ev); ++nd; }
                            }
                            ++nd;
                            a.nn_pos[p] = b.idx == INT_MAX ? -1 : b.pos;
                            a.nn_leaf[p] = b.idx == INT_MAX ? -1 : bleaf;
                            o.x = __int_as_float(0x7fc00000);
                        } else if (a.adj1_capacity > 0 && a.bvh->n_levels >= 2) {
                            const int m = (int)(__ldg(&a.node_rank[a.bvh->coffset[1] + seed_leaf + 1]) - 1u);
                            if (m < a.adj1_capacity) {
                                const float4 jlo = __ldg(&a.adj1_box[2 * (size_t)m]), jhi = __ldg(&a.adj1_box[2 * (size_t)m + 1]);
                                if (__fsub_rd(x, r) >= jlo.x && __fadd_ru(x, r) <= jhi.x && __fsub_rd(y, r) >= jlo.y &&
                                    __fadd_ru(y, r) <= jhi.y && __fsub_rd(z, r) >= jlo.z && __fadd_ru(z, r) <= jhi.z) seed.w = __int_as_float(m);
                            }
                        }
                    }
                }
            }
        }
        a.qbuf[p] = o;
        if (o.x == o.x) a.seedbuf[p] = seed;
    }
    TL_END(0);
    if (STATS) flush_stats(a, 0u, 0u, ev, nd);
}

#ifndef GROUP_CAP
#define GROUP_CAP 48
#endif
#ifndef GROUP_FRONT
#define GROUP_FRONT 64
#endif
#ifndef GROUP_WARPS
#define GROUP_WARPS 4
#endif
#ifndef GROUP_UNROLL
#define GROUP_UNROLL 3
#endif
#ifndef GROUP_STEP_LIMIT
#define GROUP_STEP_LIMIT 160
#endif
#ifndef GROUP_SIZE
#define GROUP_SIZE 32
#endif
static_assert(GROUP_CAP <= GROUP_FRONT, "pass A keeps the want masks of the listed leaves in cfirst[]");
struct GroupStage {
    unsigned int front[2][GROUP_FRONT];
    unsigned int cfirst[GROUP_FRONT], clast[GROUP_FRONT];
    float4 lo[GROUP_CAP], hi[GROUP_CAP];
    unsigned int leaf[GROUP_CAP], ls[GROUP_CAP], le[GROUP_CAP];
};
#ifdef ICP_GROUP_PROBE
__device__ unsigned long long g_group_stats[12];
extern "C" int icp_gpu_debug_group_stats(unsigned long long* out12, int reset) {
    if (reset) { void* p = nullptr; cudaGetSymbolAddress(&p, g_group_stats); return (int)cudaMemset(p, 0, sizeof(g_group_stats)); }
    return (int)cudaMemcpyFromSymbol(out12, g_group_stats, sizeof(g_group_stats));
}
#define GROUP_PROBE(x) x
#else
#define GROUP_PROBE(x)
#endif
__device__ __forceinline__ unsigned int f2ord(float f) { const unsigned int u = __float_as_uint(f); return (u & 0x80000000u) ? ~u : (u | 0x80000000u); }
__device__ __forceinline__ float ord2f(unsigned int u) { return __uint_as_float((u & 0x80000000u) ? (u & 0x7FFFFFFFu) : ~u); }
__device__ __forceinline__ float warp_min_f(float v) { return ord2f(__reduce_min_sync(0xFFFFFFFFu, f2ord(v))); }
__device__ __forceinline__ float warp_max_f(float v) { return ord2f(__reduce_max_sync(0xFFFFFFFFu, f2ord(v))); }

struct GroupBounds { float blx, bly, blz, bhx, bhy, bhz, qlx, qly, qlz, qhx, qhy, qhz, dlim; };
__device__ __forceinline__ bool group_keeps(const GroupBounds& g, const float4 lo, const float4 hi) {
    const bool meets = lo.x <= g.bhx && hi.x >= g.blx && lo.y <= g.bhy && hi.y >= g.bly && lo.z <= g.bhz && hi.z >= g.blz;
    const float gx = fmaxf(fmaxf(lo.x - g.qhx, g.qlx - hi.x), 0.0f), gy = fmaxf(fmaxf(lo.y - g.qhy, g.qly - hi.y), 0.0f), gz = fmaxf(fmaxf(lo.z - g.qhz, g.qlz - hi.z), 0.0f);
    return meets && !(gx * gx + gy * gy + gz * gz > g.dlim);
}

#define GROUP_LEFT 0xFFFFFFFFu
__device__ __forceinline__ unsigned int group_collect(const MatchArgs& a, const BvhDesc& bvh, GroupStage& sm, const Query& q, bool member, float bd, int own,
                                                      int lane, unsigned int& nd, unsigned int& n_list_out, unsigned int& scans_out) {
    const unsigned int FULL = 0xFFFFFFFFu;
    GroupBounds g;
    {
        const float INF = __int_as_float(0x7f800000);
        const float r = member ? __fmul_ru(__fsqrt_ru(bd), 1.00001f) : 0.f;
        g.blx = warp_min_f(member ? __fsub_rd(q.x, r) : INF); g.bhx = warp_max_f(member ? __fadd_ru(q.x, r) : -INF);
        g.bly = warp_min_f(member ? __fsub_rd(q.y, r) : INF); g.bhy = warp_max_f(member ? __fadd_ru(q.y, r) : -INF);
        g.blz = warp_min_f(member ? __fsub_rd(q.z, r) : INF); g.bhz = warp_max_f(member ? __fadd_ru(q.z, r) : -INF);
        g.qlx = warp_min_f(member ? q.x : INF); g.qhx = warp_max_f(member ? q.x : -INF);
        g.qly = warp_min_f(member ? q.y : INF); g.qhy = warp_max_f(member ? q.y : -INF);
        g.qlz = warp_min_f(member ? q.z : INF); g.qhz = warp_max_f(member ? q.z : -INF);
        g.dlim = __fadd_ru(__fmul_ru(warp_max_f(member ? bd : 0.f), 1.0001f), 1e-36f);
    }
    const unsigned int lt_mask = (1u << lane) - 1u;
    const int top_level = bvh.n_levels - 1;
    const unsigned int n_top = (unsigned int)bvh.count[top_level];
    unsigned int n_list = 0u, n_cur = 0u;
    int cur = 0;
    for (unsigned int base = 0; base < n_top; base += 32) {
        const unsigned int c = base + lane;
        bool keep = false; float4 lo = make_float4(0.f, 0.f, 0.f, 0.f), hi = lo; unsigned int ls = 0u, le = 0u;
        if (c < n_top) {
            lo = __ldg(&a.bvh_box[2 * (size_t)(bvh.offset[top_level] + c)]); hi = __ldg(&a.bvh_box[2 * (size_t)(bvh.offset[top_level] + c) + 1]);
            if (top_level == 0) { ls = __ldg(&a.leaf_start[c]); le = __ldg(&a.leaf_start[c + 1]); }
            keep = group_keeps(g, lo, hi);
        }
        const unsigned int mk = __ballot_sync(FULL, keep);
        if (top_level == 0) {
            if (n_list + __popc(mk) > GROUP_CAP) return GROUP_LEFT;
            if (keep) { const unsigned int k = n_list + __popc(mk & lt_mask); sm.leaf[k] = c; sm.lo[k] = lo; sm.hi[k] = hi; sm.ls[k] = ls; sm.le[k] = le; }
            n_list += __popc(mk);
        } else {
            if (n_cur + __popc(mk) > GROUP_FRONT) return GROUP_LEFT;
            if (keep) sm.front[cur][n_cur + __popc(mk & lt_mask)] = c;
            n_cur += __popc(mk);
        }
        if (lane == 0) ++nd;
    }
    __syncwarp();
    for (int L = top_level; L >= 1 && n_cur > 0u; --L) {
        for (unsigned int j = lane; j < n_cur; j += 32) {
            const unsigned int node = sm.front[cur][j];
            sm.cfirst[j] = __ldg(&a.child_start[bvh.coffset[L] + node]); sm.clast[j] = __ldg(&a.child_start[bvh.coffset[L] + node + 1]);
        }
        __syncwarp();
        const bool to_leaves = L == 1;
        const size_t box0 = (size_t)bvh.offset[L - 1];
        unsigned int n_nxt = 0u;
        for (unsigned int j0 = 0; j0 < n_cur; j0 += GROUP_UNROLL) {
            unsigned int c[GROUP_UNROLL], ls[GROUP_UNROLL], le[GROUP_UNROLL]; bool v[GROUP_UNROLL]; float4 lo[GROUP_UNROLL], hi[GROUP_UNROLL];
#pragma unroll
            for (int u = 0; u < GROUP_UNROLL; ++u) {
                v[u] = false; c[u] = 0u; ls[u] = 0u; le[u] = 0u; lo[u] = make_float4(0.f, 0.f, 0.f, 0.f); hi[u] = lo[u];
                if (j0 + u < n_cur) {
                    c[u] = sm.cfirst[j0 + u] + lane; v[u] = c[u] < sm.clast[j0 + u];
                    if (v[u]) {
                        lo[u] = __ldg(&a.bvh_box[2 * (box0 + c[u])]); hi[u] = __ldg(&a.bvh_box[2 * (box0 + c[u]) + 1]);
                        if (to_leaves) { ls[u] = __ldg(&a.leaf_start[c[u]]); le[u] = __ldg(&a.leaf_start[c[u] + 1]); }
                    }
                }
            }
#pragma unroll
            for (int u = 0; u < GROUP_UNROLL; ++u) {
                if (j0 + u >= n_cur) break;
                const bool keep = v[u] && group_keeps(g, lo[u], hi[u]);
                const unsigned int mk = __ballot_sync(FULL, keep);
                if (to_leaves) {
                    if (n_list + __popc(mk) > GROUP_CAP) return GROUP_LEFT;
                    if (keep) { const unsigned int k = n_list + __popc(mk & lt_mask); sm.leaf[k] = c[u]; sm.lo[k] = lo[u]; sm.hi[k] = hi[u]; sm.ls[k] = ls[u]; sm.le[k] = le[u]; }
                    n_list += __popc(mk);
                } else {
                    if (n_nxt + __popc(mk) > GROUP_FRONT) return GROUP_LEFT;
                    if (keep) sm.front[cur ^ 1][n_nxt + __popc(mk & lt_mask)] = c[u];
                    n_nxt += __popc(mk);
                }
                if (lane == 0) ++nd;
            }
        }
        __syncwarp();
        cur ^= 1; n_cur = n_nxt;
    }
    unsigned int scans = 0u, n_w = 0u;
    for (unsigned int j = 0; j < n_list; ++j) {
        const unsigned int leaf = sm.leaf[j];
        const bool want = member && (int)leaf != own && !(box_dist2(q, sm.lo[j], sm.hi[j]) > bd);
        const unsigned int wm = __ballot_sync(FULL, want);
        if (wm != 0u) {
            const unsigned int ls = sm.ls[j], le = sm.le[j];
            __syncwarp();
            if (lane == 0) { sm.leaf[n_w] = leaf; sm.ls[n_w] = ls; sm.le[n_w] = le; sm.cfirst[n_w] = wm; }
            ++n_w; scans += __popc(wm);
        }
    }
    __syncwarp();
    n_list_out = n_list; scans_out = scans;
    return scans > GROUP_STEP_LIMIT ? GROUP_LEFT : n_w;
}

template <bool STATS>
__global__ void __launch_bounds__(GROUP_WARPS * 32, 6) knn_group_kernel(const MatchArgs a) {
    __shared__ GroupStage s_stage[GROUP_WARPS];
    __shared__ BvhDesc s_bvh;
    if (a.desc_index < 0 && a.state_ro->converged) return;
    if (threadIdx.x < sizeof(BvhDesc) / 4) reinterpret_cast<int*>(&s_bvh)[threadIdx.x] = reinterpret_cast<const int*>(a.bvh)[threadIdx.x];
    __syncthreads();
    const unsigned int FULL = 0xFFFFFFFFu;
    const int lane = threadIdx.x & 31, wid = threadIdx.x >> 5;
    const BvhDesc& bvh = s_bvh;
    if (bvh.n_leaves <= 0) return;
    GroupStage& sm = s_stage[wid];
    const long long pl = (long long)a.q_begin + (long long)(blockIdx.x * GROUP_WARPS + wid) * GROUP_SIZE + lane;
    const int p = (int)pl;
    float4 q4 = make_float4(__int_as_float(0x7fc00000), 0.f, 0.f, 0.f), sb = make_float4(0.f, 0.f, 0.f, __int_as_float(-2));
    int own = -1;
    if (lane < GROUP_SIZE && pl < (long long)a.q_end) {
        q4 = a.qbuf[p];
        if (q4.x == q4.x) { sb = a.seedbuf[p]; own = a.nn_leaf[p]; }
    }
    const bool member = q4.x == q4.x && __float_as_int(sb.w) >= -1 && __float_as_int(sb.y) != INT_MAX;
    const int n_members = __popc(__ballot_sync(FULL, member));
    GROUP_PROBE(if (STATS && lane == 0) { atomicAdd(&g_group_stats[0], 1ull); if (n_members >= a.group_min) atomicAdd(&g_group_stats[1], 1ull); })
    if (n_members < a.group_min) return;
    GROUP_PROBE(long long t_0 = 0; long long t_2 = 0; if (STATS) t_0 = clock64();)
    Query q; q.x = q4.x; q.y = q4.y; q.z = q4.z;
    q.cr = q.cg = q.cb = 0.f;
    unsigned int ev = 0, nd = 0, n_list = 0u, scans = 0u;
    const unsigned int n_w = group_collect(a, bvh, sm, q, member, sb.x, own, lane, nd, n_list, scans);
    if (n_w == GROUP_LEFT) return;
    GROUP_PROBE(if (STATS) t_2 = clock64();)
    Best b; b.d = sb.x; b.idx = __float_as_int(sb.y); b.pos = __float_as_int(sb.z);
    int bleaf = -1;
    float4 pf[3];
#pragma unroll
    for (int u = 0; u < 3; ++u) {
        pf[u] = make_float4(0.f, 0.f, 0.f, 0.f);
        const unsigned int j = (unsigned int)u;
        if (j < n_w) {
            const unsigned int i = sm.ls[j] + lane;
            if (i < sm.le[j]) pf[u] = __ldg(&a.tgt_pts[i]);
        }
    }
    for (unsigned int j0 = 0; j0 < n_w; j0 += 3) {
#pragma unroll
        for (int u = 0; u < 3; ++u) {
            const unsigned int j = j0 + u;
            if (j >= n_w) break;
            const float4 pt = pf[u];
            if (j + 3 < n_w) {
                const unsigned int i = sm.ls[j + 3] + lane;
                if (i < sm.le[j + 3]) pf[u] = __ldg(&a.tgt_pts[i]);
            }
            const unsigned int leaf = sm.leaf[j], ls = sm.ls[j], cnt = sm.le[j] - ls;
            unsigned int wm = sm.cfirst[j];
            const bool has = (unsigned int)lane < cnt;
            const int pidx = __float_as_int(pt.w);
            while (wm) {
                const int m0 = __ffs((int)wm) - 1; wm &= wm - 1u;
                const bool two = wm != 0u;
                const int m1 = two ? __ffs((int)wm) - 1 : m0; wm &= wm - 1u;
                Query q0, q1; Best b0, b1;
                q0.x = __shfl_sync(FULL, q.x, m0); q0.y = __shfl_sync(FULL, q.y, m0); q0.z = __shfl_sync(FULL, q.z, m0);
                q1.x = __shfl_sync(FULL, q.x, m1); q1.y = __shfl_sync(FULL, q.y, m1); q1.z = __shfl_sync(FULL, q.z, m1);
                b0.d = __shfl_sync(FULL, b.d, m0); b0.idx = __shfl_sync(FULL, b.idx, m0); b0.pos = -1;
                b1.d = __shfl_sync(FULL, b.d, m1); b1.idx = __shfl_sync(FULL, b.idx, m1); b1.pos = -1;
                unsigned int key0 = 0xFFFFFFFFu, key1 = 0xFFFFFFFFu;
                if (has) {
                    key0 = __float_as_uint(dist3(q0, pt)); key1 = __float_as_uint(dist3(q1, pt));
                }
                ev += has ? (two ? 2u : 1u) : 0u;
                const unsigned int dmin0 = __reduce_min_sync(FULL, key0), dmin1 = __reduce_min_sync(FULL, key1);
                const int cand0 = (has && key0 == dmin0) ? pidx : INT_MAX, cand1 = (has && key1 == dmin1) ? pidx : INT_MAX;
                const int imin0 = __reduce_min_sync(FULL, cand0), imin1 = __reduce_min_sync(FULL, cand1);
                if (imin0 != INT_MAX && better_key(__uint_as_float(dmin0), imin0, b0)) {
                    const int src = __ffs((int)__ballot_sync(FULL, cand0 == imin0)) - 1;
                    if (lane == m0) { b.d = __uint_as_float(dmin0); b.idx = imin0; b.pos = (int)(ls + src); bleaf = (int)leaf; }
                }
                if (two && imin1 != INT_MAX && better_key(__uint_as_float(dmin1), imin1, b1)) {
                    const int src = __ffs((int)__ballot_sync(FULL, cand1 == imin1)) - 1;
                    if (lane == m1) { b.d = __uint_as_float(dmin1); b.idx = imin1; b.pos = (int)(ls + src); bleaf = (int)leaf; }
                }
            }
        }
    }
    if (member) {
        const int pos = b.idx == INT_MAX ? -1 : b.pos;
        a.nn_pos[p] = pos;
        a.nn_leaf[p] = pos >= 0 ? (bleaf >= 0 ? bleaf : own) : -1;
        a.qbuf[p].x = __int_as_float(0x7fc00000);
    }
    if (STATS) {
#ifdef ICP_GROUP_PROBE
        const long long t_3 = clock64();
        if (lane == 0) {
            atomicAdd(&g_group_stats[7], (unsigned long long)(t_2 - t_0)); atomicAdd(&g_group_stats[8], (unsigned long long)(t_3 - t_2));
            atomicMax(&g_group_stats[9], (unsigned long long)(t_3 - t_0)); atomicAdd(&g_group_stats[10], (unsigned long long)nd);
            atomicAdd(&g_group_stats[2], 1ull); atomicAdd(&g_group_stats[3], (unsigned long long)n_members);
            atomicAdd(&g_group_stats[4], (unsigned long long)n_list); atomicAdd(&g_group_stats[5], (unsigned long long)scans);
        }
#endif
        flush_stats(a, 0u, 0u, ev, nd);
    }
}

#ifndef WALK_MIN_BLOCKS
#define WALK_MIN_BLOCKS 16
#endif
template <bool COLOR, bool STATS>
__global__ void __launch_bounds__(BVH_WARPS * 32, WALK_MIN_BLOCKS) knn_bvh_kernel(const MatchArgs a) {
    __shared__ unsigned int s_node[BVH_WARPS][BVH_STACK];
    __shared__ float s_lb[BVH_WARPS][BVH_STACK];
    __shared__ BvhDesc s_bvh;
    if (a.desc_index < 0 && a.state_ro->converged) return;
    if (threadIdx.x < sizeof(BvhDesc) / 4) reinterpret_cast<int*>(&s_bvh)[threadIdx.x] = reinterpret_cast<const int*>(a.bvh)[threadIdx.x];
    __syncthreads();
    const unsigned int FULL = 0xFFFFFFFFu;
    const int lane = threadIdx.x & 31, wid = threadIdx.x >> 5;
    const int warps = (gridDim.x * blockDim.x) >> 5;
    const BvhDesc& bvh = s_bvh;
    const int top_level = bvh.n_levels - 1;
    const unsigned int n_top = (unsigned int)bvh.count[top_level];
    unsigned int ev = 0, nd = 0;
    unsigned int* st_node = s_node[wid]; float* st_lb = s_lb[wid];
    const unsigned int lt_mask = (1u << lane) - 1u;
    if (bvh.n_leaves <= 0) return;
    TL_BEGIN(1, a.state_ro->iter, a.q_begin > 0 ? 1 : 0);
    const int p0 = a.q_begin + ((blockIdx.x * blockDim.x + threadIdx.x) >> 5);
    for (int pb = p0; pb < a.q_end; pb += 32 * warps) {
      const long long pl = (long long)pb + (long long)lane * warps;
      float qx = __int_as_float(0x7fc00000);
      if (pl < (long long)a.q_end) qx = __ldg(&a.qbuf[pl].x);
      unsigned int todo = __ballot_sync(FULL, qx == qx);
      while (todo) {
        const int k = __ffs((int)todo) - 1; todo &= todo - 1u;
        const int p = pb + k * warps;
        const float4 q4 = __ldg(&a.qbuf[p]);
        Query q; q.x = q4.x; q.y = q4.y; q.z = q4.z;
        const unsigned int s_rgba = __float_as_uint(q4.w);
        q.cr = color_feature(s_rgba, 0); q.cg = color_feature(s_rgba, 1); q.cb = color_feature(s_rgba, 2);
        Best b; best_init(b, a.max_d2);
        int seed_leaf = -1;
        const float4 sb = __ldg(&a.seedbuf[p]);
        const bool handed = __float_as_int(sb.w) >= -1;
        if (handed) {
            if (lane == 0) { b.d = sb.x; b.idx = __float_as_int(sb.y); b.pos = __float_as_int(sb.z); }
        } else {
            const int sp = a.use_seed ? a.nn_pos[p] : -1;
            if (sp >= 0 && sp < a.n_tgt) {
                seed_leaf = a.nn_leaf[p];
                const unsigned int i = __ldg(&a.leaf_start[seed_leaf]) + lane;
                if (i < __ldg(&a.leaf_start[seed_leaf + 1])) {
                    const float4 c = __ldg(&a.tgt_pts[i]);
                    const float dd = dist2<COLOR>(q, c, b.d, a.tgt_nrm, i);
                    const int idx = __float_as_int(c.w);
                    if (better_key(dd, idx, b)) { b.d = dd; b.idx = idx; b.pos = (int)i; }
                    ++ev;
                }
                if (lane == 0) ++nd;
            }
        }
        bool done = false;
        if (!handed && seed_leaf >= 0 && seed_leaf < a.adj_capacity) {
            float bnd = __uint_as_float(__reduce_min_sync(FULL, __float_as_uint(b.d)));
            if (bnd < FLT_BIG) {
                const float r = __fmul_ru(__fsqrt_ru(bnd), 1.00001f);
                const float4 ilo = __ldg(&a.adj_box[2 * (size_t)seed_leaf]), ihi = __ldg(&a.adj_box[2 * (size_t)seed_leaf + 1]);
                const bool inside = __fsub_rd(q.x, r) >= ilo.x && __fadd_ru(q.x, r) <= ihi.x && __fsub_rd(q.y, r) >= ilo.y &&
                                    __fadd_ru(q.y, r) <= ihi.y && __fsub_rd(q.z, r) >= ilo.z && __fadd_ru(q.z, r) <= ihi.z;
                if (inside) {
                    const int na = __float_as_int(ilo.w);
                    unsigned int ls = 0u, le = 0u; float clb = FLT_BIG; bool keep = false;
                    if (lane < na) {
                        const unsigned int leaf = __ldg(&a.adj[(size_t)seed_leaf * 32 + lane]);
                        const float4 lo = __ldg(&a.bvh_box[2 * (size_t)leaf]), hi = __ldg(&a.bvh_box[2 * (size_t)leaf + 1]);
                        ls = __ldg(&a.leaf_start[leaf]); le = __ldg(&a.leaf_start[leaf + 1]);
                        clb = box_dist2c<COLOR>(q, lo, hi);
                        keep = !(clb > bnd);
                    }
                    if (lane == 0) ++nd;
                    bvh_scan_leaves<COLOR>(a, q, b, bnd, ls, le, clb, keep, lane, ev, nd);
                    done = true;
                }
            }
        }
        if (!done && (handed ? __float_as_int(sb.w) >= 0 : seed_leaf >= 0) && top_level >= 1 && a.adj1_capacity > 0) {
            const int m = handed ? __float_as_int(sb.w) : (int)(__ldg(&a.node_rank[bvh.coffset[1] + seed_leaf + 1]) - 1u);
            float bnd = __uint_as_float(__reduce_min_sync(FULL, __float_as_uint(b.d)));
            if (m < a.adj1_capacity && bnd < FLT_BIG) {
                const float4 ilo = __ldg(&a.adj1_box[2 * (size_t)m]);
                bool inside = true;
                if (!handed) {
                    const float r = __fmul_ru(__fsqrt_ru(bnd), 1.00001f);
                    const float4 ihi = __ldg(&a.adj1_box[2 * (size_t)m + 1]);
                    inside = __fsub_rd(q.x, r) >= ilo.x && __fadd_ru(q.x, r) <= ihi.x && __fsub_rd(q.y, r) >= ilo.y &&
                             __fadd_ru(q.y, r) <= ihi.y && __fsub_rd(q.z, r) >= ilo.z && __fadd_ru(q.z, r) <= ihi.z;
                }
                if (inside) {
                    const int na = __float_as_int(ilo.w);
                    unsigned int node = 0; unsigned int key = 0xFFFFFFFFu;
                    unsigned int cfirst = 0u, clast = 0u;
                    if (lane < na) {
                        node = __ldg(&a.adj1[(size_t)m * 32 + lane]);
                        cfirst = __ldg(&a.child_start[bvh.coffset[1] + node]); clast = __ldg(&a.child_start[bvh.coffset[1] + node + 1]);
                        const float clb = box_dist2c<COLOR>(q, __ldg(&a.bvh_box[2 * (size_t)(bvh.offset[1] + node)]), __ldg(&a.bvh_box[2 * (size_t)(bvh.offset[1] + node) + 1]));
                        if (!(clb > bnd)) key = __float_as_uint(clb);
                    }
                    if (lane == 0) ++nd;
                    int top = 0;
                    for (;;) {
                        const unsigned int kmin = __reduce_min_sync(FULL, key);
                        if (kmin == 0xFFFFFFFFu || __uint_as_float(kmin) > bnd) break;
                        const int src = __ffs((int)__ballot_sync(FULL, key == kmin)) - 1;
                        const unsigned int first = __shfl_sync(FULL, cfirst, src), last = __shfl_sync(FULL, clast, src);
                        if (lane == src) key = 0xFFFFFFFFu;
                        if (lane == 0) ++nd;
                        bvh_visit<COLOR>(a, bvh, q, b, bnd, 0, first, last, st_node, st_lb, top, lane, lt_mask, ev, nd);
                    }
                    done = true;
                }
            }
        }
        if (!done && !__any_sync(FULL, b.pos >= 0) && top_level > 0) {
            int L = top_level; unsigned int first = 0, last = n_top;
            unsigned int best_node = 0;
            for (;;) {
                unsigned int kbest = 0xFFFFFFFFu; best_node = first;
                for (unsigned int base = first; base < last; base += 32) {
                    const unsigned int c = base + lane;
                    unsigned int key = 0xFFFFFFFFu;
                    if (c < last) {
                        const float4 lo = __ldg(&a.bvh_box[2 * (size_t)(bvh.offset[L] + c)]), hi = __ldg(&a.bvh_box[2 * (size_t)(bvh.offset[L] + c) + 1]);
                        key = __float_as_uint(box_dist2c<COLOR>(q, lo, hi));
                    }
                    const unsigned int kmin = __reduce_min_sync(FULL, key);
                    if (kmin < kbest) { kbest = kmin; best_node = base + (unsigned int)(__ffs((int)__ballot_sync(FULL, key == kmin)) - 1); }
                }
                if (L == 0) break;
                first = __ldg(&a.child_start[bvh.coffset[L] + best_node]); last = __ldg(&a.child_start[bvh.coffset[L] + best_node + 1]);
                --L;
            }
            const unsigned int i = __ldg(&a.leaf_start[best_node]) + lane;
            if (i < __ldg(&a.leaf_start[best_node + 1])) {
                const float4 c = __ldg(&a.tgt_pts[i]);
                const float dd = dist2<COLOR>(q, c, b.d, a.tgt_nrm, i);
                const int idx = __float_as_int(c.w);
                if (better_key(dd, idx, b)) { b.d = dd; b.idx = idx; b.pos = (int)i; }
                ++ev;
            }
        }
        float bound = __uint_as_float(__reduce_min_sync(FULL, __float_as_uint(b.d)));
        int top = 0;
        for (unsigned int base = 0; base < n_top && !done; base += 32) {
            bvh_visit<COLOR>(a, bvh, q, b, bound, top_level, base, min(base + 32u, n_top), st_node, st_lb, top, lane, lt_mask, ev, nd);
            if (lane == 0) ++nd;
            while (top > 0) {
                --top;
                const unsigned int nd_id = st_node[top]; const float nlb = st_lb[top];
                __syncwarp();
                if (nlb > bound) continue;
                const int lvl = (int)(nd_id >> 27); const unsigned int j = nd_id & 0x7FFFFFFu;
                if (lane == 0) ++nd;
                const unsigned int first = __ldg(&a.child_start[bvh.coffset[lvl] + j]), last = __ldg(&a.child_start[bvh.coffset[lvl] + j + 1]);
                bvh_visit<COLOR>(a, bvh, q, b, bound, lvl - 1, first, last, st_node, st_lb, top, lane, lt_mask, ev, nd);
            }
        }
        const unsigned int dmin = __reduce_min_sync(FULL, __float_as_uint(b.d));
        const int cand = (__float_as_uint(b.d) == dmin) ? b.idx : INT_MAX;
        const int imin = __reduce_min_sync(FULL, cand);
        const int src_lane = __ffs((int)__ballot_sync(FULL, cand == imin)) - 1;
        const int pos = imin == INT_MAX ? -1 : __shfl_sync(FULL, b.pos, src_lane);
        if (lane == 0) {
            a.nn_pos[p] = pos;
            a.nn_leaf[p] = pos >= 0 ? (int)(__ldg(&a.leaf_rank[pos + 1]) - 1u) : -1;
        }
      }
    }
    TL_END(1);
    if (STATS) flush_stats(a, 0u, 0u, ev, nd);
}

__global__ void __launch_bounds__(256) match_finish_kernel(const MatchArgs a) {
    __shared__ PoseSm sm;
    if (a.desc_index < 0 && a.state_ro->converged) return;
    load_pose(sm, a.state_ro);
    const IterDesc d = a.desc[a.desc_index >= 0 ? a.desc_index : a.state_ro->iter];
    const int p = blockIdx.x * blockDim.x + threadIdx.x;
    unsigned int nq = 0, nm = 0;
    if (p < a.n_src) {
        Query q; float snx, sny, snz; unsigned int s_rgba;
        if (prepare_query(a, d, sm, p, q, snx, sny, snz, s_rgba)) {
            ++nq;
            int pos = finite3(q.x, q.y, q.z) ? a.nn_pos[p] : -1;
            if (pos >= a.n_tgt) pos = -1;
            const int idx = pos >= 0 ? __float_as_int(__ldg(&a.tgt_pts[pos].w)) : -1;
            finish_match(a, p, pos >= 0, 1.0f, idx, pos, q.x, q.y, q.z, snx, sny, snz, s_rgba, nm);
        } else {
            write_no_query(a, p);
        }
    }
    flush_stats(a, nq, nm, 0u, 0u);
}

template <bool COLOR, bool NORM>
__global__ void __launch_bounds__(ICP_MATCH_THREADS) knn_brute_kernel(const MatchArgs a) {
    __shared__ PoseSm sm;
    if (a.desc_index < 0 && a.state_ro->converged) return;
    load_pose(sm, a.state_ro);
    const IterDesc d = a.desc[a.desc_index >= 0 ? a.desc_index : a.state_ro->iter];
    const int lane = threadIdx.x & 31;
    const int p = (blockIdx.x * blockDim.x + threadIdx.x) >> 5;
    unsigned int nq = 0, nm = 0, ev = 0, nd = 0;
    if (p < a.n_src) {
        Query q; float snx, sny, snz; unsigned int s_rgba;
        if (prepare_query(a, d, sm, p, q, snx, sny, snz, s_rgba)) {
            Best b; b.d = fminf(a.max_d2, FLT_BIG); b.idx = INT_MAX; b.pos = -1;
            if (finite3(q.x, q.y, q.z)) {
                for (int j = lane; j < a.n_tgt; j += 32) {
                    const float4 c = __ldg(&a.tgt_pts[j]);
                    float dd = dist2<COLOR>(q, c, b.d, a.tgt_nrm, (unsigned int)j);
                    if (NORM) dd = __fsqrt_rn(dist3(q, c));
                    if (better(dd, j, b)) { b.d = dd; b.idx = j; b.pos = j; }
                }
                ev += (unsigned int)((a.n_tgt - lane + 31) / 32);
#pragma unroll
                for (int o = 16; o > 0; o >>= 1) {
                    Best t; t.d = __shfl_xor_sync(0xFFFFFFFFu, b.d, o); t.idx = __shfl_xor_sync(0xFFFFFFFFu, b.idx, o); t.pos = t.idx;
                    if (better(t.d, t.idx, b)) b = t;
                }
                if (b.idx == INT_MAX) b.pos = -1; else b.pos = b.idx;
            }
            if (lane == 0) { ++nq; finish_match(a, p, b.pos >= 0, 1.0f, b.idx, b.pos, q.x, q.y, q.z, snx, sny, snz, s_rgba, nm); }
        } else if (lane == 0) {
            write_no_query(a, p);
        }
    }
    flush_stats(a, nq, nm, ev, nd);
}

#define PROJ_TILE_MAX 2800
template <int PROJ_THREADS, int TILE_MAX, int MIN_BLOCKS>
__global__ void __launch_bounds__(PROJ_THREADS, MIN_BLOCKS) projective_kernel(const MatchArgs a) {
    __shared__ PoseSm sm;
    __shared__ float4 tile[TILE_MAX];
    __shared__ unsigned int s_box[4][PROJ_THREADS / 32];
    if (a.desc_index < 0 && a.state_ro->converged) return;
    load_pose(sm, a.state_ro);
    const IterDesc d = a.desc[a.desc_index >= 0 ? a.desc_index : a.state_ro->iter];
    const int lane = threadIdx.x & 31, wid = threadIdx.x >> 5;
    int p; bool in;
    if (a.proj_tiled) {
        const unsigned int tiles_x = (a.width + 31u) / 32u;
        const unsigned int u = (blockIdx.x % tiles_x) * 32u + (unsigned int)lane, v = (blockIdx.x / tiles_x) * (PROJ_THREADS / 32) + (unsigned int)wid;
        in = u < a.width && v < a.height;
        p = (int)(v * a.width + u);
    } else {
        p = blockIdx.x * blockDim.x + threadIdx.x;
        in = p < a.n_src;
    }
    const unsigned int searchWindow = 12u;
    unsigned int nq = 0, nm = 0, ev = 0, nd = 0;
    Query q; float snx = 0.f, sny = 0.f, snz = 0.f; unsigned int s_rgba = 0;
    q.x = q.y = q.z = 0.f; q.cr = q.cg = q.cb = 0.f;
    const bool is_query = in && prepare_query(a, d, sm, p, q, snx, sny, snz, s_rgba);
    const bool scans = is_query && !(q.x == MINF_F);
    unsigned int uP = 0, vP = 0, u0 = 0xFFFFFFFFu, v0 = 0xFFFFFFFFu, u1 = 0, v1 = 0;
    bool has_window = false;
    if (scans) {
        uP = x86_float_to_u32(roundf(padd(pdiv(pmul(q.x, a.fx), q.z), a.cx)));
        vP = x86_float_to_u32(roundf(padd(pdiv(pmul(q.y, a.fy), q.z), a.cy)));
        const unsigned int vs = vP - searchWindow, us = uP - searchWindow;
        if (vs < a.height && us < a.width && vs <= vP + searchWindow && us <= uP + searchWindow) {
            has_window = true;
            u0 = us; v0 = vs;
            u1 = min(uP + searchWindow, a.width - 1u); v1 = min(vP + searchWindow, a.height - 1u);
        }
    }
    unsigned int bu0 = __reduce_min_sync(0xFFFFFFFFu, u0), bv0 = __reduce_min_sync(0xFFFFFFFFu, v0);
    unsigned int bu1 = __reduce_max_sync(0xFFFFFFFFu, has_window ? u1 : 0u), bv1 = __reduce_max_sync(0xFFFFFFFFu, has_window ? v1 : 0u);
    if (lane == 0) { s_box[0][wid] = bu0; s_box[1][wid] = bv0; s_box[2][wid] = bu1; s_box[3][wid] = bv1; }
    __syncthreads();
#pragma unroll
    for (int w = 0; w < PROJ_THREADS / 32; ++w) { bu0 = min(bu0, s_box[0][w]); bv0 = min(bv0, s_box[1][w]); bu1 = max(bu1, s_box[2][w]); bv1 = max(bv1, s_box[3][w]); }
    const bool any_window = bu0 != 0xFFFFFFFFu;
    const unsigned int tw = any_window ? bu1 - bu0 + 1u : 0u, th = any_window ? bv1 - bv0 + 1u : 0u;
    const unsigned int tp = (tw + 7u) & ~7u;
    const bool staged = any_window && (unsigned long long)tp * th <= TILE_MAX;
    if (any_window && !staged && threadIdx.x == 0) ++nd;
    if (staged) {
        for (unsigned int k = threadIdx.x; k < tw * th; k += PROJ_THREADS) {
            const unsigned int ty = k / tw, tx = k - ty * tw;
            tile[ty * tp + tx] = __ldg(&a.tgt_pts[(size_t)a.width * (bv0 + ty) + bu0 + tx]);
        }
    }
    __syncthreads();
    if (in) {
        if (!is_query) write_no_query(a, p);
        else {
            ++nq;
            if (!scans) {
                finish_match(a, p, true, 0.0f, 0, 0, q.x, q.y, q.z, snx, sny, snz, s_rgba, nm);
            } else {
                float minDist = FLT_BIG; unsigned int idx = 0xFFFFFFFFu;
                if (has_window) {
                    const unsigned int n_u = u1 - u0 + 1u;
                    unsigned int cnt = 0u, best = 0xFFFFFFFFu;
                    if (staged) {
                        const float4* row = &tile[(v0 - bv0) * tp + (u0 - bu0)];
                        for (unsigned int v = v0; v <= v1; ++v, row += tp) {
#pragma unroll 5
                            for (unsigned int k = 0; k < n_u; ++k, ++cnt) {
                                const float4 t = row[k];
                                const float dx = psub(q.x, t.x), dy = psub(q.y, t.y), dz = psub(q.z, t.z);
                                const float dist = padd(padd(pmul(dx, dx), pmul(dy, dy)), pmul(dz, dz));
                                if (minDist > dist) { best = cnt; minDist = dist; }
                            }
                        }
                    } else {
                        const float4* row = &a.tgt_pts[(size_t)a.width * v0 + u0];
                        for (unsigned int v = v0; v <= v1; ++v, row += a.width) {
#pragma unroll 5
                            for (unsigned int k = 0; k < n_u; ++k, ++cnt) {
                                const float4 t = __ldg(&row[k]);
                                const float dx = psub(q.x, t.x), dy = psub(q.y, t.y), dz = psub(q.z, t.z);
                                const float dist = padd(padd(pmul(dx, dx), pmul(dy, dy)), pmul(dz, dz));
                                if (minDist > dist) { best = cnt; minDist = dist; }
                            }
                        }
                    }
                    ev += cnt;
                    if (best != 0xFFFFFFFFu) idx = a.width * (v0 + best / n_u) + u0 + best % n_u;
                }
                const bool ok = minDist <= a.max_d2 && idx != 0xFFFFFFFFu;
                finish_match(a, p, ok, 1.0f, (int)idx, (int)idx, q.x, q.y, q.z, snx, sny, snz, s_rgba, nm);
            }
        }
    }
    flush_stats(a, nq, nm, ev, nd);
}

cudaError_t icp_launch_match(const MatchArgs& a, int algorithm, int n_sms, cudaStream_t s, int* n_launches, cudaEvent_t after_prep,
                             const MatchChunks* chunks) {
    if (a.n_src <= 0) return cudaSuccess;
    const int T = ICP_MATCH_THREADS;
    int launches = 0;
    if (algorithm == 2) {
        static const bool no_small = getenv("ICP_GPU_NO_SMALL_PROJ_BLOCKS") != nullptr;
        if (!a.proj_tiled && a.n_src < 2 * 256 * n_sms && !no_small) {
            projective_kernel<64, PROJ_TILE_MAX, 5><<<(unsigned int)((a.n_src + 63) / 64), 64, 0, s>>>(a);
        } else if (a.proj_tiled) {
            const unsigned int nb = ((a.width + 31u) / 32u) * ((a.height + 128 / 32 - 1u) / (128 / 32));
            projective_kernel<128, 2304, 6><<<nb, 128, 0, s>>>(a);
        } else {
            projective_kernel<256, PROJ_TILE_MAX, 5><<<(unsigned int)((a.n_src + 256 - 1) / 256), 256, 0, s>>>(a);
        }
        ++launches;
    } else if (algorithm == 1) {
        const long long threads = (long long)a.n_src * 32;
        const int nb = (int)((threads + T - 1) / T);
        if (a.color_icp) knn_brute_kernel<true, false><<<nb, T, 0, s>>>(a);
        else if (a.brute_norm) knn_brute_kernel<false, true><<<nb, T, 0, s>>>(a);
        else knn_brute_kernel<false, false><<<nb, T, 0, s>>>(a);
        ++launches;
    } else {
        int K = (chunks && !after_prep) ? chunks->n : 1;
        if (K < 1) K = 1;
        long long per = ((long long)a.n_src + K - 1) / K;
        per = (per + 255) / 256 * 256;
        if (K > 1) cudaEventRecord(chunks->fork, s);
        static const int mult = getenv("ICP_GPU_WALK_GRID") ? atoi(getenv("ICP_GPU_WALK_GRID")) : 64;
        for (int c = 0; c < K; ++c) {
            MatchArgs ac = a;
            ac.q_begin = (int)std::min<long long>((long long)c * per, a.n_src);
            ac.q_end = (int)std::min<long long>((long long)(c + 1) * per, a.n_src);
            const int nq = ac.q_end - ac.q_begin;
            if (nq <= 0) continue;
            cudaStream_t cs = c == 0 ? s : chunks->stream[c - 1];
            if (c > 0) cudaStreamWaitEvent(cs, chunks->fork, 0);
            const int np = (nq + PREP_THREADS - 1) / PREP_THREADS;
            if (a.collect_stats) { if (a.color_icp) knn_prep_kernel<true, true><<<np, PREP_THREADS, 0, cs>>>(ac); else knn_prep_kernel<false, true><<<np, PREP_THREADS, 0, cs>>>(ac); }
            else { if (a.color_icp) knn_prep_kernel<true, false><<<np, PREP_THREADS, 0, cs>>>(ac); else knn_prep_kernel<false, false><<<np, PREP_THREADS, 0, cs>>>(ac); }
            ++launches;
            if (after_prep) cudaEventRecord(after_prep, s);
            const int group_min = getenv("ICP_GPU_GROUP_MIN") ? atoi(getenv("ICP_GPU_GROUP_MIN")) : (a.max_d2 >= 1.0f ? 8 : 0);
            if (group_min > 0 && a.fast_path && a.use_seed && !a.color_icp) {
                ac.group_min = group_min;
                const int ng = (nq + GROUP_SIZE * GROUP_WARPS - 1) / (GROUP_SIZE * GROUP_WARPS);
                if (a.collect_stats) knn_group_kernel<true><<<ng, GROUP_WARPS * 32, 0, cs>>>(ac); else knn_group_kernel<false><<<ng, GROUP_WARPS * 32, 0, cs>>>(ac);
                ++launches;
            }
            int nb = (nq + BVH_WARPS - 1) / BVH_WARPS;
            const int cap = std::max(1, mult * n_sms * 4 / BVH_WARPS);
            if (nb > cap) nb = cap;
            if (a.collect_stats) { if (a.color_icp) knn_bvh_kernel<true, true><<<nb, BVH_WARPS * 32, 0, cs>>>(ac); else knn_bvh_kernel<false, true><<<nb, BVH_WARPS * 32, 0, cs>>>(ac); }
            else { if (a.color_icp) knn_bvh_kernel<true, false><<<nb, BVH_WARPS * 32, 0, cs>>>(ac); else knn_bvh_kernel<false, false><<<nb, BVH_WARPS * 32, 0, cs>>>(ac); }
            ++launches;
            if (c > 0) { cudaEventRecord(chunks->done[c - 1], cs); cudaStreamWaitEvent(s, chunks->done[c - 1], 0); }
        }
        if (!a.skip_finish) { match_finish_kernel<<<(a.n_src + 255) / 256, 256, 0, s>>>(a); ++launches; }
    }
    if (n_launches) *n_launches += launches;
    return cudaGetLastError();
}
```

### icp_variants_b200/csrc/registration.cu

```cuda
#include "context.cuh"
#include <stdlib.h>

namespace {

struct Mt19937 {
    uint32_t mt[624]; int idx;
    void seed(uint32_t s) {
        mt[0] = s;
        for (int i = 1; i < 624; ++i) mt[i] = 1812433253u * (mt[i - 1] ^ (mt[i - 1] >> 30)) + (uint32_t)i;
        idx = 624;
    }
    uint32_t next() {
        if (idx >= 624) {
            for (int i = 0; i < 624; ++i) {
                const uint32_t y = (mt[i] & 0x80000000u) | (mt[(i + 1) % 624] & 0x7fffffffu);
                mt[i] = mt[(i + 397) % 624] ^ (y >> 1) ^ ((y & 1u) ? 0x9908b0dfu : 0u);
            }
            idx = 0;
        }
        uint32_t y = mt[idx++];
        y ^= (y >> 11); y ^= (y << 7) & 0x9d2c5680u; y ^= (y << 15) & 0xefc60000u; y ^= (y >> 18);
        return y;
    }
    double canonical() {
        const double lo = (double)next(), hi = (double)next();
        double v = (lo + hi * 4294967296.0) / 18446744073709551616.0;
        if (v >= 1.0) v = nextafter(1.0, 0.0);
        return v;
    }
};

long long __float_as_int_host(float f) { int32_t i; memcpy(&i, &f, 4); return (long long)i; }

struct Plan {
    int n_iters = 0;
    std::vector<IterDesc> desc;
    std::vector<uint32_t> mask;
    std::vector<int> voxel_depth;
};

struct KernelClouds { const float4 *src_pts, *src_nrm, *tgt_pts, *tgt_nrm; bool tiled; };

}

void draw_selection_masks(const icp_gpu_config& cfg, const IcpSchedule& sch, long long n, const uint8_t* finite, uint32_t* out) {
    const size_t words = mask_words(n);
    Mt19937 rng; int level = -1;
    for (int i = 0; i < sch.n_iters; ++i) {
        const int lv = icp_schedule_level(sch, i), stride = icp_schedule_stride(sch, i);
        if (lv != level) { rng.seed(cfg.seed + (uint32_t)lv); level = lv; }
        uint32_t* m = out + (size_t)i * words;
        for (long long k = 0; k < n; k += stride) {
            if (cfg.multires && !finite[(size_t)k]) continue;
            if (rng.canonical() < cfg.proba) m[k >> 5] |= 1u << (k & 31);
        }
    }
}

int choose_algorithm(const icp_gpu_ctx* c) {
    if (c->cfg.matching == ICP_GPU_MATCH_PROJECTIVE) return 2;
    if (c->cfg.nn_algorithm == ICP_GPU_NN_BRUTE || c->cfg.nn_algorithm == ICP_GPU_NN_BRUTE_NORM) return 1;
    if (c->cfg.nn_algorithm == ICP_GPU_NN_GRID) return 0;
    return c->n_tgt <= 2048 ? 1 : 0;
}

int check_ready(icp_gpu_ctx* ctx) {
    if (ctx->n_src < 0) return fail(ctx, ICP_GPU_E_STATE, "no source cloud set");
    if (ctx->n_tgt < 0) return fail(ctx, ICP_GPU_E_STATE, "no target cloud set (buildIndex)");
    if (ctx->cfg.matching == ICP_GPU_MATCH_PROJECTIVE) {
        if (!ctx->have_camera) return fail(ctx, ICP_GPU_E_STATE, "projective matching needs icp_gpu_set_camera");
        if ((long long)ctx->width * ctx->height != (long long)ctx->n_tgt || ctx->height == 0)
            return fail(ctx, ICP_GPU_E_STATE, "projective matching: target size %d != width*height %u*%u", ctx->n_tgt, ctx->width, ctx->height);
    }
    return 0;
}

static int make_plan(icp_gpu_ctx* ctx, Plan& plan) {
    const icp_gpu_config& cfg = ctx->cfg;
    const int n = ctx->n_src;
    const bool host_rng = cfg.selection == ICP_GPU_SELECT_RANDOM && cfg.selection_rng == ICP_GPU_RNG_MT19937;
    const bool dev_rng = cfg.selection == ICP_GPU_SELECT_RANDOM && cfg.selection_rng == ICP_GPU_RNG_DEVICE;
    if (host_rng && cfg.multires && fetch_src_finite(ctx)) return ICP_GPU_E_CUDA;
    const size_t words = mask_words(n);
    const bool voxel = cfg.multires && cfg.pyramid_mode == ICP_GPU_PYRAMID_VOXEL;
    const IcpSchedule sch = icp_schedule(cfg.n_iterations, cfg.multires, n);
    if (sch.n_iters > ICP_MAX_ITERS) return fail(ctx, ICP_GPU_E_ARG, "more than %d iterations", ICP_MAX_ITERS);
    if (host_rng) {
        plan.mask.assign((size_t)sch.n_iters * words, 0u);
        draw_selection_masks(cfg, sch, n, ctx->src_finite.data(), plan.mask.data());
    }
    for (int i = 0; i < sch.n_iters; ++i) {
        const int stride = icp_schedule_stride(sch, i);
        IterDesc d = all_points_desc();
        d.stride = stride; d.filter_finite = cfg.multires ? 1 : 0;
        if (voxel && stride > 1) {
            int k = 0; while ((1 << k) < stride) ++k;
            int D = (ctx->Ts < 22 ? ctx->Ts : 22) - (3 * k + 1) / 2; if (D < 0) D = 0;
            int slot = -1;
            for (size_t j = 0; j < plan.voxel_depth.size(); ++j) if (plan.voxel_depth[j] == D) slot = (int)j;
            if (slot < 0) { slot = (int)plan.voxel_depth.size(); plan.voxel_depth.push_back(D); }
            d.stride = 1; d.mask_word_offset = (int)((size_t)slot * words);
        }
        if (dev_rng) { d.proba = (float)cfg.proba; d.rng_key = cfg.seed * 2654435761u + (uint32_t)(i + 1) * 0x9E3779B9u; }
        if (host_rng) d.mask_word_offset = (int)((size_t)i * words);
        plan.desc.push_back(d);
    }
    plan.n_iters = sch.n_iters;
    return 0;
}

static bool proj_tiled(const icp_gpu_ctx* c, int algo) {
    return algo == 2 && c->n_src > 0 && (long long)c->width * c->height == (long long)c->n_src && !getenv("ICP_GPU_NO_PROJ_TILES");
}

static KernelClouds kernel_clouds(const icp_gpu_ctx* c, int algo) {
    const bool grid_order = algo == 0, tiled = proj_tiled(c, algo);
    return {(const float4*)(tiled ? c->src_raw_pts.p : c->src_pts.p), (const float4*)(tiled ? c->src_raw_nrm.p : c->src_nrm.p),
            (const float4*)(grid_order ? c->tgt_pts_sorted.p : c->tgt_pts.p), (const float4*)(grid_order ? c->tgt_nrm_sorted.p : c->tgt_nrm.p), tiled};
}

void fill_match_args(icp_gpu_ctx* c, MatchArgs& a, int algo, int desc_index, bool want_idx) {
    memset(&a, 0, sizeof(a));
    const KernelClouds k = kernel_clouds(c, algo);
    a.src_pts = k.src_pts; a.src_nrm = k.src_nrm; a.n_src = c->n_src; a.proj_tiled = k.tiled ? 1 : 0;
    a.mask = (const unsigned int*)c->mask.p; a.desc = (const IterDesc*)c->desc.p;
    a.state_ro = (const DevState*)c->state.p; a.state = (DevState*)c->state.p;
    a.tgt_pts = k.tgt_pts; a.tgt_nrm = k.tgt_nrm; a.n_tgt = c->n_tgt;
    a.bvh_box = (const float4*)c->bvh_box.p; a.bvh = (const BvhDesc*)c->bvh_desc.p; a.leaf_start = (const unsigned int*)c->leaf_start.p;
    a.leaf_rank = (const unsigned int*)c->leaf_rank.p; a.child_start = (const unsigned int*)c->child_start.p;
    a.adj = (const unsigned int*)c->adj.p; a.adj_box = (const float4*)c->adj_box.p; a.adj_capacity = c->adj_capacity;
    a.adj_gap = getenv("ICP_GPU_NO_ADJ_GAP") ? nullptr : (const float*)c->adj_gap.p;
    a.nn_leaf = (int*)c->nn_leaf.p;
    a.adj1 = (const unsigned int*)c->adj1.p; a.adj1_box = (const float4*)c->adj1_box.p; a.adj1_capacity = c->adj1_capacity;
    a.node_rank = (const unsigned int*)c->node_rank.p;
    if (getenv("ICP_GPU_NO_ADJACENCY1")) a.adj1_capacity = 0;
    if (getenv("ICP_GPU_NO_ADJACENCY")) a.adj_capacity = 0;
    if (c->have_camera) { a.fx = c->K[0]; a.fy = c->K[4]; a.cx = c->K[6]; a.cy = c->K[7]; }
    a.width = c->width; a.height = c->height;
    a.weighting = c->cfg.weighting; a.rejection = c->cfg.rejection; a.color_icp = c->cfg.color_icp;
    a.max_d2 = c->cfg.max_distance_sq;
    a.weight_max_d2 = c->cfg.weight_max_distance_sq > 0.f ? c->cfg.weight_max_distance_sq : c->cfg.max_distance_sq;
    a.match_pos = (int*)c->match_pos.p; a.match_w = (float*)c->match_w.p; a.match_idx = want_idx ? (int*)c->match_idx.p : nullptr;
    a.nn_pos = (int*)c->nn_pos.p; a.qbuf = (float4*)c->qbuf.p; a.seedbuf = (float4*)c->seedbuf.p;
    a.desc_index = desc_index;
    a.q_begin = 0; a.q_end = c->n_src;
    a.use_seed = algo == 0 ? 1 : 0;
    a.brute_norm = c->cfg.nn_algorithm == ICP_GPU_NN_BRUTE_NORM ? 1 : 0;
    a.fast_path = getenv("ICP_GPU_NO_FASTPATH") ? 0 : 1;
    a.collect_stats = c->cfg.collect_stats;
}

void fill_reduce_args(icp_gpu_ctx* c, ReduceArgs& r, int algo, int solve) {
    memset(&r, 0, sizeof(r));
    const KernelClouds k = kernel_clouds(c, algo);
    r.src_pts = k.src_pts; r.src_nrm = k.src_nrm; r.n_src = c->n_src;
    r.state = (DevState*)c->state.p;
    r.tgt_pts = k.tgt_pts; r.tgt_nrm = k.tgt_nrm;
    r.match_pos = (const int*)c->match_pos.p; r.match_w = (const float*)c->match_w.p;
    r.partials = (double*)c->partials.p; r.pose_history = (float*)c->history.p;
    r.metric = c->cfg.metric; r.solve = solve;
    r.fused = 0; r.nn_pos = (const int*)c->nn_pos.p; r.n_tgt = c->n_tgt; r.mask = (const unsigned int*)c->mask.p;
    r.desc = (const IterDesc*)c->desc.p; r.desc_index = -1;
    r.weighting = c->cfg.weighting; r.rejection = c->cfg.rejection; r.max_d2 = c->cfg.max_distance_sq;
    r.weight_max_d2 = c->cfg.weight_max_distance_sq > 0.f ? c->cfg.weight_max_distance_sq : c->cfg.max_distance_sq;
    r.profile = getenv("ICP_GPU_REDUCE_PROFILE") ? 1 : 0;
    if (solve && c->peer_world > 1) {
        r.peer.world = c->peer_world; r.peer.rank = c->peer_rank;
        unsigned long long ms = 2000;
        if (const char* e = getenv("ICP_GPU_PEER_TIMEOUT_MS")) { const long long v = atoll(e); if (v >= 1 && v <= 600000) ms = (unsigned long long)v; }
        r.peer.timeout_ns = ms * 1000000ull;
        for (int j = 0; j < c->peer_world; ++j) r.peer.box[j] = (PeerBox*)c->peer_ptr[j];
        r.peer.plan_check = c->peer_plan_check;
    }
}

int refresh_seeds(icp_gpu_ctx* ctx, int algo, bool allow_seed) {
    if (algo != 0 || ctx->n_src <= 0 || !ctx->nn_pos.p) return 0;
    const bool seed = allow_seed && ctx->n_tgt > 0 && ctx->grid_built && !getenv("ICP_GPU_NO_GRID_SEED");
    if (seed) {
        CU(icp_launch_seed_from_keys((const float4*)ctx->src_pts.p, ctx->n_src, (const DevState*)ctx->state.p, (const GridParams*)ctx->grid.p,
                                     ctx->tsort.keys_sorted, ctx->n_tgt, (const unsigned int*)ctx->bbox.p + 7, (const unsigned int*)ctx->tsort.msd.p,
                                     ctx->tsort.msd_shift, (const unsigned int*)ctx->leaf_rank.p, (int*)ctx->nn_pos.p, (int*)ctx->nn_leaf.p,
                                     ctx->nn_stale ? 1 : 0, ctx->stream));
        ctx->stats.n_kernel_launches += 1;
    } else if (ctx->nn_stale) {
        CU(icp_launch_fill_int((int*)ctx->nn_pos.p, ctx->n_src, -1, ctx->stream));
        ctx->stats.n_kernel_launches += 1;
    }
    ctx->nn_stale = false;
    return 0;
}

static int enqueue_iterations(icp_gpu_ctx* ctx, const Plan& plan, int algo, std::vector<cudaEvent_t>* ev_marks) {
    MatchArgs ma; ReduceArgs ra;
    fill_match_args(ctx, ma, algo, -1, false);
    fill_reduce_args(ctx, ra, algo, 1);
    if (algo == 0 && ctx->cfg.minimizer == ICP_GPU_MIN_LINEAR && !ctx->cfg.collect_stats) { ma.skip_finish = 1; ra.fused = 1; }
    int launches = 0;
    const int nb = ctx->n_reduce_blocks;
    MatchChunks mc = ctx->chunks;
    mc.n = ctx->n_src >= 131072 ? 2 : 1;
    if (const char* e = getenv("ICP_GPU_MATCH_CHUNKS")) { const int v = atoi(e); if (v >= 1 && v <= ICP_MAX_MATCH_CHUNKS) mc.n = v; }
    for (int i = 0; i < plan.n_iters; ++i) {
        if (ev_marks) CU(cudaEventRecord((*ev_marks)[2 * i], ctx->stream));
        CU(icp_launch_match(ma, algo, ctx->n_sms, ctx->stream, &launches, (ev_marks && algo == 0) ? (*ev_marks)[2 * plan.n_iters + 1 + i] : nullptr, &mc));
        if (ev_marks) CU(cudaEventRecord((*ev_marks)[2 * i + 1], ctx->stream));
        if (ctx->cfg.minimizer == ICP_GPU_MIN_LM) CU(icp_launch_lm(ra, nb, ctx->cfg.lm_max_iterations, ctx->stream, &launches));
        else CU(icp_launch_reduce(ra, nb, ctx->stream, &launches));
    }
    if (ev_marks) CU(cudaEventRecord((*ev_marks)[2 * plan.n_iters], ctx->stream));
    ctx->stats.n_kernel_launches += (uint64_t)launches;
    return 0;
}

static int start_registration(icp_gpu_ctx* ctx, const float pose_in[16], icp_gpu_timings* timings) {
    if (!pose_in) return ICP_GPU_E_ARG;
    if (int rc = enter(ctx)) return rc;
    int rc = check_ready(ctx); if (rc) return rc;
    if (join_index(ctx)) return ICP_GPU_E_CUDA;
    if (ctx->peer_world > 1 && ctx->cfg.multires)
        return fail(ctx, ICP_GPU_E_ARG, "point-sharded registration: the multi-resolution schedule is derived from the local shard (level strides and count "
                                        "differ between ranks and from the unsharded cloud); run it with multires off");
    Plan plan;
    rc = make_plan(ctx, plan); if (rc) return rc;
    ctx->peer_plan_check = plan.n_iters * 64 + ctx->cfg.metric * 16 + ctx->cfg.minimizer * 8 + (ctx->cfg.lm_max_iterations & 7);
    const int algo = choose_algorithm(ctx);
    memset(&ctx->stats, 0, sizeof(ctx->stats));
    memcpy(ctx->h_desc, plan.desc.data(), sizeof(IterDesc) * (size_t)plan.n_iters);
    if (plan.n_iters > 0) CU(cudaMemcpyAsync(ctx->desc.p, ctx->h_desc, sizeof(IterDesc) * (size_t)plan.n_iters, cudaMemcpyHostToDevice, ctx->stream));
    if (!plan.voxel_depth.empty()) {
        const size_t words = mask_words(ctx->n_src);
        int dmax = 0; for (int D : plan.voxel_depth) dmax = D > dmax ? D : dmax;
        if (ensure(ctx, ctx->mask, plan.voxel_depth.size() * words * sizeof(uint32_t)) ||
            ensure(ctx, ctx->voxel_table, sizeof(unsigned int) * ((size_t)1 << dmax))) return ICP_GPU_E_CUDA;
        int launches = 0;
        for (size_t j = 0; j < plan.voxel_depth.size(); ++j)
            CU(icp_launch_voxel_level((const float4*)ctx->src_pts.p, (const float4*)ctx->src_nrm.p, ctx->n_src, (const GridParams*)ctx->sgrid.p,
                                      ctx->Ts, plan.voxel_depth[j], (unsigned int*)ctx->voxel_table.p, (unsigned int*)ctx->mask.p + j * words,
                                      words, ctx->stream, &launches));
        ctx->stats.n_kernel_launches += (uint64_t)launches;
    }
    if (!plan.mask.empty()) {
        if (ensure(ctx, ctx->mask, plan.mask.size() * sizeof(uint32_t))) return ICP_GPU_E_CUDA;
        CU(cudaMemcpyAsync(ctx->mask.p, plan.mask.data(), plan.mask.size() * sizeof(uint32_t), cudaMemcpyHostToDevice, ctx->stream));
        CU(cudaStreamSynchronize(ctx->stream));
    }
    if (upload_pose(ctx, pose_in, ctx->cfg.early_stop_rotation, ctx->cfg.early_stop_translation)) return ICP_GPU_E_CUDA;
    ctx->stats.n_kernel_launches += 1;
    rc = refresh_seeds(ctx, algo, true); if (rc) return rc;

    std::vector<cudaEvent_t> marks;
    if (timings) {
        memset(timings, 0, sizeof(*timings));
        marks.resize((size_t)3 * plan.n_iters + 1);
        for (auto& e : marks) CU(cudaEventCreate(&e));
        rc = enqueue_iterations(ctx, plan, algo, &marks);
    } else if (ctx->cfg.use_graph && plan.n_iters > 0) {
        std::vector<long long> key;
        key.push_back(algo); key.push_back(ctx->cfg.metric); key.push_back(ctx->cfg.minimizer); key.push_back(ctx->cfg.lm_max_iterations);
        key.push_back(ctx->cfg.weighting); key.push_back(ctx->cfg.rejection); key.push_back(ctx->cfg.color_icp); key.push_back(ctx->cfg.collect_stats);
        key.push_back((long long)__float_as_int_host(ctx->cfg.max_distance_sq)); key.push_back((long long)__float_as_int_host(ctx->cfg.weight_max_distance_sq));
        key.push_back(ctx->n_src); key.push_back(ctx->n_tgt); key.push_back(ctx->T); key.push_back(ctx->width); key.push_back(ctx->height);
        for (int k = 0; k < 9; ++k) key.push_back((long long)__float_as_int_host(ctx->have_camera ? ctx->K[k] : 0.f));
        key.push_back((long long)(uintptr_t)ctx->mask.p); key.push_back((long long)(uintptr_t)ctx->stream);
        key.push_back(plan.n_iters);
        key.push_back(ctx->peer_world); key.push_back(ctx->peer_rank); key.push_back((long long)ctx->peer_epoch);
        if (!ctx->graph_exec || key != ctx->graph_key) {
            cudaGraph_t g = nullptr;
            CU(cudaStreamBeginCapture(ctx->stream, cudaStreamCaptureModeThreadLocal));
            const uint64_t before = ctx->stats.n_kernel_launches;
            rc = enqueue_iterations(ctx, plan, algo, nullptr);
            cudaError_t ce = cudaStreamEndCapture(ctx->stream, &g);
            if (rc) { if (g) cudaGraphDestroy(g); return rc; }
            if (ce != cudaSuccess) return fail(ctx, ICP_GPU_E_CUDA, "cudaStreamEndCapture: %s", cudaGetErrorString(ce));
            bool updated = false;
            if (ctx->graph_exec) {
                cudaGraphExecUpdateResultInfo info;
                updated = cudaGraphExecUpdate(ctx->graph_exec, g, &info) == cudaSuccess;
                if (!updated) { cudaGetLastError(); cudaGraphExecDestroy(ctx->graph_exec); ctx->graph_exec = nullptr; }
            }
            ce = updated ? cudaSuccess : cudaGraphInstantiate(&ctx->graph_exec, g, 0);
            cudaGraphDestroy(g);
            if (ce != cudaSuccess) { ctx->graph_exec = nullptr; return fail(ctx, ICP_GPU_E_CUDA, "cudaGraphInstantiate: %s", cudaGetErrorString(ce)); }
            ctx->graph_key = key;
            ctx->graph_launches = ctx->stats.n_kernel_launches - before;
        } else {
            ctx->stats.n_kernel_launches += ctx->graph_launches;
        }
        CU(cudaGraphLaunch(ctx->graph_exec, ctx->stream));
    } else {
        rc = enqueue_iterations(ctx, plan, algo, nullptr);
    }
    if (rc) return rc;
    CU(cudaMemcpyAsync(ctx->h_state, ctx->state.p, sizeof(DevState), cudaMemcpyDeviceToHost, ctx->stream));
    if (plan.n_iters > 0) CU(cudaMemcpyAsync(ctx->h_history, ctx->history.p, sizeof(float) * 16 * (size_t)plan.n_iters, cudaMemcpyDeviceToHost, ctx->stream));
    ctx->pending = true; ctx->pending_iters = plan.n_iters;
    if (timings) {
        CU(cudaStreamSynchronize(ctx->stream));
        for (int i = 0; i < plan.n_iters; ++i) {
            float a = 0.f, b = 0.f;
            cudaEventElapsedTime(&a, marks[2 * i], marks[2 * i + 1]);
            cudaEventElapsedTime(&b, marks[2 * i + 1], marks[2 * i + 2]);
            timings->matching_ms += a; timings->solver_ms += b;
            float c = 0.f;
            if (algo == 0 && cudaEventElapsedTime(&c, marks[2 * i], marks[2 * plan.n_iters + 1 + i]) == cudaSuccess) timings->search_prep_ms += c; else cudaGetLastError();
        }
        float tot = 0.f;
        if (plan.n_iters > 0) cudaEventElapsedTime(&tot, marks[0], marks[2 * plan.n_iters]);
        float idx_ms = 0.f;
        if (ctx->grid_built && cudaEventElapsedTime(&idx_ms, ctx->ev[0], ctx->ev[1]) == cudaSuccess) ctx->index_ms = idx_ms; else cudaGetLastError();
        timings->total_ms = tot; timings->index_ms = ctx->index_ms; timings->n_iterations = plan.n_iters;
        const int per_match = algo == 0 ? ((ctx->cfg.minimizer == ICP_GPU_MIN_LINEAR && !ctx->cfg.collect_stats) ? 2 : 3) : 1;
        timings->n_match_launches = plan.n_iters * per_match;
        timings->n_solver_launches = (int)ctx->stats.n_kernel_launches - 1 - plan.n_iters * per_match;
        for (auto& e : marks) cudaEventDestroy(e);
    }
    return ICP_GPU_OK;
}

static void copy_counters(icp_gpu_ctx* ctx) {
    const DevState& st = *ctx->h_state;
    ctx->stats.n_queries = st.n_queries; ctx->stats.n_matched = st.n_matched;
    ctx->stats.n_distance_evals = st.n_evals; ctx->stats.n_nodes_visited = st.n_nodes;
    for (int k = 0; k < 6; ++k) ctx->stats.reduce_profile_ns[k] = st.prof[k];
}

int icp_gpu_estimate_pose_finish(icp_gpu_ctx* ctx, float pose_out[16], float* pose_history, int32_t* n_iterations_out) {
    if (int rc = enter(ctx, false)) return rc;
    if (!ctx->pending) return fail(ctx, ICP_GPU_E_STATE, "no registration pending");
    ctx->pending = false;
    CU(cudaStreamSynchronize(ctx->stream));
    const DevState& st = *ctx->h_state;
    if (pose_out) memcpy(pose_out, st.pose, 16 * sizeof(float));
    if (pose_history && st.iters_done > 0) memcpy(pose_history, ctx->h_history, sizeof(float) * 16 * (size_t)st.iters_done);
    if (n_iterations_out) *n_iterations_out = st.iters_done;
    ctx->last_iters = st.iters_done;
    copy_counters(ctx);
    return status_error(ctx, st.status, st.iters_done, "iteration %d had no surviving correspondence (the reference hangs in ASSERT here)");
}

int icp_gpu_query_matches(icp_gpu_ctx* ctx, const float pose[16], const int32_t* sel_idx, int64_t n_sel, int32_t* idx_out, float* weight_out) {
    if (!pose || !idx_out || !weight_out) return ICP_GPU_E_ARG;
    if (int rc = enter(ctx)) return rc;
    int rc = check_ready(ctx); if (rc) return rc;
    if (join_index(ctx)) return ICP_GPU_E_CUDA;
    const int n = ctx->n_src;
    const int nq = sel_idx ? (int)n_sel : n;
    if (sel_idx && (n_sel < 0 || n_sel > n)) return fail(ctx, ICP_GPU_E_ARG, "n_sel %lld", (long long)n_sel);
    memset(&ctx->stats, 0, sizeof(ctx->stats));
    if (fetch_src_rank(ctx)) return ICP_GPU_E_CUDA;
    IterDesc d = all_points_desc();
    std::vector<uint32_t> mask;
    if (sel_idx) {
        mask.assign(mask_words(n), 0u);
        for (int64_t k = 0; k < n_sel; ++k) {
            if (sel_idx[k] < 0 || sel_idx[k] >= n) return fail(ctx, ICP_GPU_E_ARG, "sel_idx[%lld] out of range", (long long)k);
            mask[(size_t)sel_idx[k] >> 5] |= 1u << (sel_idx[k] & 31);
        }
        if (ensure(ctx, ctx->mask, mask.size() * 4)) return ICP_GPU_E_CUDA;
        CU(cudaMemcpyAsync(ctx->mask.p, mask.data(), mask.size() * 4, cudaMemcpyHostToDevice, ctx->stream));
        d.mask_word_offset = 0;
    }
    ctx->h_desc[DESC_QUERY] = d;
    CU(cudaMemcpyAsync((IterDesc*)ctx->desc.p + DESC_QUERY, &ctx->h_desc[DESC_QUERY], sizeof(IterDesc), cudaMemcpyHostToDevice, ctx->stream));
    if (upload_pose(ctx, pose)) return ICP_GPU_E_CUDA;
    const int algo = choose_algorithm(ctx);
    rc = refresh_seeds(ctx, algo, false); if (rc) return rc;
    MatchArgs ma; fill_match_args(ctx, ma, algo, DESC_QUERY, true);
    int launches = 1;
    CU(icp_launch_match(ma, algo, ctx->n_sms, ctx->stream, &launches));
    ctx->stats.n_kernel_launches += (uint64_t)launches;
    std::vector<int> idx_s((size_t)n); std::vector<float> w_s((size_t)n);
    if (n > 0) {
        CU(cudaMemcpyAsync(idx_s.data(), ctx->match_idx.p, (size_t)n * 4, cudaMemcpyDeviceToHost, ctx->stream));
        CU(cudaMemcpyAsync(w_s.data(), ctx->match_w.p, (size_t)n * 4, cudaMemcpyDeviceToHost, ctx->stream));
    }
    CU(cudaMemcpyAsync(ctx->h_state, ctx->state.p, sizeof(DevState), cudaMemcpyDeviceToHost, ctx->stream));
    CU(cudaStreamSynchronize(ctx->stream));
    for (int k = 0; k < nq; ++k) {
        const int o = sel_idx ? sel_idx[k] : k;
        const int p = ma.proj_tiled ? o : ctx->src_rank[(size_t)o];
        idx_out[k] = idx_s[(size_t)p]; weight_out[k] = w_s[(size_t)p];
    }
    copy_counters(ctx);
    return ICP_GPU_OK;
}

int icp_gpu_iterations_bound(const icp_gpu_config* cfg, int64_t n_source) {
    if (!cfg || n_source < 0 || n_source > 0x7fffffff) return ICP_GPU_E_ARG;
    return icp_schedule(cfg->n_iterations, cfg->multires, n_source).n_iters;
}

int icp_gpu_max_iterations(const icp_gpu_ctx* ctx) {
    if (!ctx) return ICP_GPU_E_ARG;
    return icp_gpu_iterations_bound(&ctx->cfg, ctx->n_src > 0 ? ctx->n_src : 0);
}

int icp_gpu_estimate_pose_async(icp_gpu_ctx* ctx, const float pose_in[16]) { return start_registration(ctx, pose_in, nullptr); }

int icp_gpu_estimate_pose(icp_gpu_ctx* ctx, float pose_inout[16], float* pose_history, int32_t* n_iterations_out, icp_gpu_timings* timings) {
    if (int rc = start_registration(ctx, pose_inout, timings)) return rc;
    return icp_gpu_estimate_pose_finish(ctx, pose_inout, pose_history, n_iterations_out);
}
```

### profiles/probe_timeline.py

```python
import ctypes as C
import json
import os
import sys

import numpy as np
import torch

os.environ.setdefault("ICP_GPU_LIB_NAME", "libicp_gpu_timeline.so")
sys.path.insert(0, os.path.dirname(os.path.dirname(os.path.abspath(__file__))))
from icp_variants_b200 import capi, synth

TL_WARPS = 40960


def resident(starts, ends, t_grid):
    s = np.sort(starts); e = np.sort(ends)
    return np.searchsorted(s, t_grid, side="right") - np.searchsorted(e, t_grid, side="right")


def main():
    torch.cuda.set_device(0)
    lib = C.CDLL(capi.LIB_PATH)
    ctx = capi.Context(0)
    stream = torch.cuda.Stream()
    torch.cuda.set_stream(stream)
    ctx.set_stream(stream.cuda_stream)
    src, tgt, _ = synth.eth_pair(seed=1234)
    cfg = capi.default_config()
    cfg.metric, cfg.minimizer, cfg.matching, cfg.n_iterations, cfg.max_distance_sq, cfg.nn_algorithm, cfg.collect_stats = 1, 0, 0, 30, 10.0, 2, 0
    ctx.set_config(cfg)
    for rep in range(4):
        ctx.set_target(tgt.points, tgt.normals, tgt.colors)
        ctx.set_source(src.points, src.normals, src.colors)
        torch.cuda.synchronize()
        if rep == 3:
            lib.icp_gpu_debug_timeline(None, 1)
            lib.icp_gpu_debug_timeline_reduce(None, 1)
            torch.cuda.synchronize()
        ctx.estimate_pose(want_history=False)
        torch.cuda.synchronize()
    tl = np.zeros((2, 2, TL_WARPS, 2), np.uint64)
    tr = np.zeros((512, 2), np.uint64)
    lib.icp_gpu_debug_timeline(tl.ctypes.data_as(C.c_void_p), 0)
    lib.icp_gpu_debug_timeline_reduce(tr.ctypes.data_as(C.c_void_p), 0)
    tl = tl.astype(np.int64); tr = tr.astype(np.int64)
    t0 = tl[0][tl[0][:, :, 0] > 0][:, 0].min()
    out = {"chunks": os.environ.get("ICP_GPU_MATCH_CHUNKS", "default"), "unit": "microseconds from the iteration's first prep warp", "kernels": {}}
    spans = {}
    for k, name in ((0, "prep"), (1, "walk")):
        for c in range(2):
            w = tl[k, c]; w = w[w[:, 0] > 0]
            if len(w) == 0:
                continue
            s = (w[:, 0] - t0) * 1e-3; e = (w[:, 1] - t0) * 1e-3
            life = e - s
            spans[f"{name}{c}"] = (s, e)
            out["kernels"][f"{name}_chunk{c}"] = {
                "warps": int(len(w)), "first_start": round(float(s.min()), 2), "last_start": round(float(s.max()), 2), "end": round(float(e.max()), 2),
                "warp_life_us": {"mean": round(float(life.mean()), 2), "p50": round(float(np.median(life)), 2), "p90": round(float(np.percentile(life, 90)), 2),
                                 "p99": round(float(np.percentile(life, 99)), 2), "max": round(float(life.max()), 2)},
                "time_when_95pct_of_warps_had_ended": round(float(np.percentile(e, 95)), 2),
            }
    b = tr[:511]; b = b[b[:, 0] > 0]
    out["kernels"]["reduce"] = {"blocks": int(len(b)), "first_start": round(float((b[:, 0].min() - t0) * 1e-3), 2),
                                "loops_end": round(float((b[:, 1].max() - t0) * 1e-3), 2), "pose_written": round(float((tr[511, 0] - t0) * 1e-3), 2)}
    end = out["kernels"]["reduce"]["pose_written"]
    grid = np.arange(0.0, end + 5.0, 5.0)
    tot = {}
    for name, (s, e) in spans.items():
        tot[name] = resident(s, e, grid) / 148.0
    out["resident_warps_per_sm_every_5us"] = {name: [round(float(x), 1) for x in v] for name, v in tot.items()}
    print(json.dumps(out))


if __name__ == "__main__":
    main()
```

Before: 219.5.

## Precompute group membership masks in prep and optionally run group kernel on side stream

The prep kernel now writes a per-warp-window membership bitmask, so the group kernel can skip empty windows without loading query data. An opt-in mode (ICP_GPU_GROUP_BESIDE) runs the group kernel plus a leftover walk over abandoned windows on a separate stream, while the main BVH walk handles only points outside the group mask. This is meant to overlap the two search paths instead of running them serially. The side-stream mode is off by default, so by default only the mask precompute and early-exit path change behaviour.

```diff
diff --git a/icp_variants_b200/csrc/clouds.cu b/icp_variants_b200/csrc/clouds.cu
--- a/icp_variants_b200/csrc/clouds.cu
+++ b/icp_variants_b200/csrc/clouds.cu
@@ -137,7 +137,8 @@
         const size_t n1 = (size_t)(n > 0 ? n : 1);
         if (ensure(ctx, ctx->match_pos, n1 * 4) || ensure(ctx, ctx->match_w, n1 * 4) || ensure(ctx, ctx->match_idx, n1 * 4) ||
             ensure(ctx, ctx->nn_pos, n1 * 4) || ensure(ctx, ctx->nn_leaf, n1 * 4) || ensure(ctx, ctx->qbuf, n1 * sizeof(float4)) ||
-            ensure(ctx, ctx->seedbuf, n1 * sizeof(float4))) return ICP_GPU_E_CUDA;
+            ensure(ctx, ctx->seedbuf, n1 * sizeof(float4)) || ensure(ctx, ctx->group_mask, (n1 + 31) / 32 * 4) ||
+            ensure(ctx, ctx->group_left, ((n1 + 31) / 32 + ICP_MAX_MATCH_CHUNKS) * 4)) return ICP_GPU_E_CUDA;
         ctx->n_reduce_blocks = icp_reduce_blocks((int)n, ctx->n_sms);
         if (ensure(ctx, ctx->partials, (size_t)ctx->n_reduce_blocks * ICP_NRED * sizeof(double))) return ICP_GPU_E_CUDA;
         if (build_source(ctx)) return ICP_GPU_E_CUDA;
diff --git a/icp_variants_b200/csrc/context.cu b/icp_variants_b200/csrc/context.cu
--- a/icp_variants_b200/csrc/context.cu
+++ b/icp_variants_b200/csrc/context.cu
@@ -121,6 +121,10 @@
         ok = ok && cudaStreamCreateWithFlags(&ctx->chunks.stream[c], cudaStreamNonBlocking) == cudaSuccess &&
              cudaEventCreateWithFlags(&ctx->chunks.done[c], cudaEventDisableTiming) == cudaSuccess;
     ok = ok && cudaEventCreateWithFlags(&ctx->chunks.fork, cudaEventDisableTiming) == cudaSuccess;
+    for (int c = 0; c < ICP_MAX_MATCH_CHUNKS; ++c)
+        ok = ok && cudaStreamCreateWithFlags(&ctx->chunks.group_stream[c], cudaStreamNonBlocking) == cudaSuccess &&
+             cudaEventCreateWithFlags(&ctx->chunks.group_fork[c], cudaEventDisableTiming) == cudaSuccess &&
+             cudaEventCreateWithFlags(&ctx->chunks.group_done[c], cudaEventDisableTiming) == cudaSuccess;
     for (int i = 0; ok && i < 4; ++i) ok = cudaEventCreate(&ctx->ev[i]) == cudaSuccess;
     for (int i = 0; ok && i < 2; ++i) ok = cudaEventCreateWithFlags(&ctx->ev_xyz[i], cudaEventDisableTiming) == cudaSuccess && cudaEventCreateWithFlags(&ctx->ev_copied[i], cudaEventDisableTiming) == cudaSuccess &&
                                            cudaEventCreateWithFlags(&ctx->ev_packed[i], cudaEventDisableTiming) == cudaSuccess;
@@ -157,6 +161,11 @@
         if (ctx->chunks.stream[c]) { cudaStreamSynchronize(ctx->chunks.stream[c]); cudaStreamDestroy(ctx->chunks.stream[c]); }
     for (int c = 0; c < ICP_MAX_MATCH_CHUNKS - 1; ++c) if (ctx->chunks.done[c]) cudaEventDestroy(ctx->chunks.done[c]);
     if (ctx->chunks.fork) cudaEventDestroy(ctx->chunks.fork);
+    for (int c = 0; c < ICP_MAX_MATCH_CHUNKS; ++c) {
+        if (ctx->chunks.group_stream[c]) { cudaStreamSynchronize(ctx->chunks.group_stream[c]); cudaStreamDestroy(ctx->chunks.group_stream[c]); }
+        if (ctx->chunks.group_fork[c]) cudaEventDestroy(ctx->chunks.group_fork[c]);
+        if (ctx->chunks.group_done[c]) cudaEventDestroy(ctx->chunks.group_done[c]);
+    }
     if (ctx->ev_index_ready) cudaEventDestroy(ctx->ev_index_ready);
     if (ctx->aux_stream) cudaStreamDestroy(ctx->aux_stream);
     if (ctx->copy_stream) cudaStreamDestroy(ctx->copy_stream);
diff --git a/icp_variants_b200/csrc/context.cuh b/icp_variants_b200/csrc/context.cuh
--- a/icp_variants_b200/csrc/context.cuh
+++ b/icp_variants_b200/csrc/context.cuh
@@ -45,7 +45,7 @@
     bool nn_stale = true;
     DeviceBuf sgrid, sbbox, order_dev, voxel_table;
     int Ts = 0;
-    DeviceBuf state, desc, mask, match_pos, match_w, match_idx, nn_pos, nn_leaf, qbuf, seedbuf, partials, pose_dev, history;
+    DeviceBuf state, desc, mask, match_pos, match_w, match_idx, nn_pos, nn_leaf, qbuf, seedbuf, group_mask, group_left, partials, pose_dev, history;
     DeviceBuf nrm_out_dev;
     DeviceBuf prep_in, prep_tmp, prep_out, gt_src, gt_ref, met_partial, met_out;
     DeviceBuf scratch[16];
diff --git a/icp_variants_b200/csrc/icp_internal.cuh b/icp_variants_b200/csrc/icp_internal.cuh
--- a/icp_variants_b200/csrc/icp_internal.cuh
+++ b/icp_variants_b200/csrc/icp_internal.cuh
@@ -148,6 +148,8 @@
     int skip_finish;
     int q_begin, q_end;
     int group_min;
+    unsigned int* group_mask;
+    int* group_left;
 };
 
 #define ICP_MAX_MATCH_CHUNKS 8
@@ -156,6 +158,9 @@
     cudaStream_t stream[ICP_MAX_MATCH_CHUNKS - 1] = {};
     cudaEvent_t done[ICP_MAX_MATCH_CHUNKS - 1] = {};
     cudaEvent_t fork = nullptr;
+    int group_beside = 0;
+    cudaStream_t group_stream[ICP_MAX_MATCH_CHUNKS] = {};
+    cudaEvent_t group_fork[ICP_MAX_MATCH_CHUNKS] = {}, group_done[ICP_MAX_MATCH_CHUNKS] = {};
 };
 
 struct ReduceArgs {
diff --git a/icp_variants_b200/csrc/match.cu b/icp_variants_b200/csrc/match.cu
--- a/icp_variants_b200/csrc/match.cu
+++ b/icp_variants_b200/csrc/match.cu
@@ -110,7 +110,7 @@
 #ifdef ICP_TIMELINE
 #define ICP_TL_ITER 12
 #define ICP_TL_WARPS 40960
-__device__ unsigned long long g_timeline[2][2][ICP_TL_WARPS][2];
+__device__ unsigned long long g_timeline[4][2][ICP_TL_WARPS][2];
 __device__ __forceinline__ unsigned long long tl_now() { unsigned long long t; asm volatile("mov.u64 %0, %%globaltimer;" : "=l"(t)); return t; }
 extern "C" int icp_gpu_debug_timeline(unsigned long long* out, int reset) {
     if (reset) { void* p = nullptr; cudaGetSymbolAddress(&p, g_timeline); return (int)cudaMemset(p, 0, sizeof(g_timeline)); }
@@ -218,6 +218,7 @@
 #ifndef PREP_THREADS
 #define PREP_THREADS 256
 #endif
+static_assert(PREP_THREADS % 32 == 0, "a prep warp is one window of group_mask");
 #ifndef PREP_MIN_BLOCKS
 #define PREP_MIN_BLOCKS 5
 #endif
@@ -237,6 +238,7 @@
     load_pose(sm, a.state_ro);
     const IterDesc d = a.desc[desc_i];
     unsigned int ev = 0, nd = 0;
+    bool member = false;
     if (p < a.q_end) {
         float4 o = make_float4(__int_as_float(0x7fc00000), 0.f, 0.f, n4.w);
         float4 seed = make_float4(0.f, 0.f, 0.f, __int_as_float(-2));
@@ -296,6 +298,13 @@
         }
         a.qbuf[p] = o;
         if (o.x == o.x) a.seedbuf[p] = seed;
+        member = o.x == o.x && __float_as_int(seed.w) >= -1 && __float_as_int(seed.y) != INT_MAX;
+        if (a.group_left) member = member && __float_as_int(seed.w) >= 0;
+    }
+    if (a.group_min > 0) {
+        const unsigned int mk = __ballot_sync(0xFFFFFFFFu, member);
+        if ((threadIdx.x & 31) == 0 && p < a.q_end) a.group_mask[p >> 5] = __popc(mk) >= (unsigned int)a.group_min ? mk : 0u;
+        if (a.group_left && blockIdx.x == 0 && threadIdx.x == 0) a.group_left[0] = 0;
     }
     TL_END(0);
     if (STATS) flush_stats(a, 0u, 0u, ev, nd);
@@ -316,9 +325,7 @@
 #ifndef GROUP_STEP_LIMIT
 #define GROUP_STEP_LIMIT 160
 #endif
-#ifndef GROUP_SIZE
 #define GROUP_SIZE 32
-#endif
 static_assert(GROUP_CAP <= GROUP_FRONT, "pass A keeps the want masks of the listed leaves in cfirst[]");
 struct GroupStage {
     unsigned int front[2][GROUP_FRONT];
@@ -461,24 +468,29 @@
     const BvhDesc& bvh = s_bvh;
     if (bvh.n_leaves <= 0) return;
     GroupStage& sm = s_stage[wid];
-    const long long pl = (long long)a.q_begin + (long long)(blockIdx.x * GROUP_WARPS + wid) * GROUP_SIZE + lane;
-    const int p = (int)pl;
+    const int win = (a.q_begin >> 5) + (int)(blockIdx.x * GROUP_WARPS + wid);
+    const int p = win * GROUP_SIZE + lane;
+    const unsigned int owned = ((long long)win * GROUP_SIZE < (long long)a.q_end) ? __ldg(&a.group_mask[win]) : 0u;
+    GROUP_PROBE(if (STATS && lane == 0) { atomicAdd(&g_group_stats[0], 1ull); if (owned) atomicAdd(&g_group_stats[1], 1ull); })
+    if (owned == 0u) return;
+    TL_BEGIN(2, a.state_ro->iter, a.q_begin > 0 ? 1 : 0);
+    const bool member = (owned >> lane) & 1u;
+    const int n_members = __popc(owned);
     float4 q4 = make_float4(__int_as_float(0x7fc00000), 0.f, 0.f, 0.f), sb = make_float4(0.f, 0.f, 0.f, __int_as_float(-2));
     int own = -1;
-    if (lane < GROUP_SIZE && pl < (long long)a.q_end) {
-        q4 = a.qbuf[p];
-        if (q4.x == q4.x) { sb = a.seedbuf[p]; own = a.nn_leaf[p]; }
-    }
-    const bool member = q4.x == q4.x && __float_as_int(sb.w) >= -1 && __float_as_int(sb.y) != INT_MAX;
-    const int n_members = __popc(__ballot_sync(FULL, member));
-    GROUP_PROBE(if (STATS && lane == 0) { atomicAdd(&g_group_stats[0], 1ull); if (n_members >= a.group_min) atomicAdd(&g_group_stats[1], 1ull); })
-    if (n_members < a.group_min) return;
+    if (member) {
+        q4 = a.qbuf[p]; sb = a.seedbuf[p]; own = a.nn_leaf[p];
+    }
     GROUP_PROBE(long long t_0 = 0; long long t_2 = 0; if (STATS) t_0 = clock64();)
     Query q; q.x = q4.x; q.y = q4.y; q.z = q4.z;
     q.cr = q.cg = q.cb = 0.f;
     unsigned int ev = 0, nd = 0, n_list = 0u, scans = 0u;
     const unsigned int n_w = group_collect(a, bvh, sm, q, member, sb.x, own, lane, nd, n_list, scans);
-    if (n_w == GROUP_LEFT) return;
+    if (n_w == GROUP_LEFT) {
+        if (a.group_left && lane == 0) a.group_left[1 + atomicAdd(&a.group_left[0], 1)] = win;
+        TL_END(2);
+        return;
+    }
     GROUP_PROBE(if (STATS) t_2 = clock64();)
     Best b; b.d = sb.x; b.idx = __float_as_int(sb.y); b.pos = __float_as_int(sb.z);
     int bleaf = -1;
@@ -538,8 +550,9 @@
         const int pos = b.idx == INT_MAX ? -1 : b.pos;
         a.nn_pos[p] = pos;
         a.nn_leaf[p] = pos >= 0 ? (bleaf >= 0 ? bleaf : own) : -1;
-        a.qbuf[p].x = __int_as_float(0x7fc00000);
-    }
+        if (!a.group_left) a.qbuf[p].x = __int_as_float(0x7fc00000);
+    }
+    TL_END(2);
     if (STATS) {
 #ifdef ICP_GROUP_PROBE
         const long long t_3 = clock64();
@@ -554,10 +567,11 @@
     }
 }
 
+enum WalkPart { WALK_ALL = 0, WALK_UNOWNED = 1, WALK_LEFT = 2 };
 #ifndef WALK_MIN_BLOCKS
 #define WALK_MIN_BLOCKS 16
 #endif
-template <bool COLOR, bool STATS>
+template <int PART, bool COLOR, bool STATS>
 __global__ void __launch_bounds__(BVH_WARPS * 32, WALK_MIN_BLOCKS) knn_bvh_kernel(const MatchArgs a) {
     __shared__ unsigned int s_node[BVH_WARPS][BVH_STACK];
     __shared__ float s_lb[BVH_WARPS][BVH_STACK];
@@ -575,16 +589,25 @@
     unsigned int* st_node = s_node[wid]; float* st_lb = s_lb[wid];
     const unsigned int lt_mask = (1u << lane) - 1u;
     if (bvh.n_leaves <= 0) return;
-    TL_BEGIN(1, a.state_ro->iter, a.q_begin > 0 ? 1 : 0);
-    const int p0 = a.q_begin + ((blockIdx.x * blockDim.x + threadIdx.x) >> 5);
-    for (int pb = p0; pb < a.q_end; pb += 32 * warps) {
+    TL_BEGIN(PART == WALK_LEFT ? 3 : 1, a.state_ro->iter, a.q_begin > 0 ? 1 : 0);
+    const int p0 = (PART == WALK_LEFT ? 0 : a.q_begin) + ((blockIdx.x * blockDim.x + threadIdx.x) >> 5);
+    const int p_end = PART == WALK_LEFT ? 32 * a.group_left[0] : a.q_end;
+    for (int pb = p0; pb < p_end; pb += 32 * warps) {
       const long long pl = (long long)pb + (long long)lane * warps;
-      float qx = __int_as_float(0x7fc00000);
-      if (pl < (long long)a.q_end) qx = __ldg(&a.qbuf[pl].x);
-      unsigned int todo = __ballot_sync(FULL, qx == qx);
+      bool search = false;
+      if (PART == WALK_LEFT) {
+        if (pl < (long long)p_end)
+          search = (__ldg(&a.group_mask[a.group_left[1 + (int)(pl >> 5)]]) >> (pl & 31)) & 1u;
+      } else if (pl < (long long)a.q_end) {
+        const float qx = __ldg(&a.qbuf[pl].x);
+        search = qx == qx;
+        if (PART == WALK_UNOWNED) search = search && !((__ldg(&a.group_mask[pl >> 5]) >> (pl & 31)) & 1u);
+      }
+      unsigned int todo = __ballot_sync(FULL, search);
       while (todo) {
         const int k = __ffs((int)todo) - 1; todo &= todo - 1u;
-        const int p = pb + k * warps;
+        const int v = pb + k * warps;
+        const int p = PART == WALK_LEFT ? a.group_left[1 + (v >> 5)] * 32 + (v & 31) : v;
         const float4 q4 = __ldg(&a.qbuf[p]);
         Query q; q.x = q4.x; q.y = q4.y; q.z = q4.z;
         const unsigned int s_rgba = __float_as_uint(q4.w);
@@ -726,8 +749,19 @@
         }
       }
     }
-    TL_END(1);
+    TL_END(PART == WALK_LEFT ? 3 : 1);
     if (STATS) flush_stats(a, 0u, 0u, ev, nd);
+}
+
+template <int PART>
+static void launch_walk(const MatchArgs& a, int nb, cudaStream_t s) {
+    if constexpr (PART == WALK_ALL) {
+        if (a.color_icp) {
+            if (a.collect_stats) knn_bvh_kernel<PART, true, true><<<nb, BVH_WARPS * 32, 0, s>>>(a); else knn_bvh_kernel<PART, true, false><<<nb, BVH_WARPS * 32, 0, s>>>(a);
+            return;
+        }
+    }
+    if (a.collect_stats) knn_bvh_kernel<PART, false, true><<<nb, BVH_WARPS * 32, 0, s>>>(a); else knn_bvh_kernel<PART, false, false><<<nb, BVH_WARPS * 32, 0, s>>>(a);
 }
 
 __global__ void __launch_bounds__(256) match_finish_kernel(const MatchArgs a) {
@@ -919,6 +953,9 @@
         per = (per + 255) / 256 * 256;
         if (K > 1) cudaEventRecord(chunks->fork, s);
         static const int mult = getenv("ICP_GPU_WALK_GRID") ? atoi(getenv("ICP_GPU_WALK_GRID")) : 64;
+        const int group_min = getenv("ICP_GPU_GROUP_MIN") ? atoi(getenv("ICP_GPU_GROUP_MIN")) : (a.max_d2 >= 1.0f ? 8 : 0);
+        const bool group_on = group_min > 0 && a.fast_path && a.use_seed && !a.color_icp;
+        const bool beside = group_on && chunks && chunks->group_beside;
         for (int c = 0; c < K; ++c) {
             MatchArgs ac = a;
             ac.q_begin = (int)std::min<long long>((long long)c * per, a.n_src);
@@ -927,24 +964,30 @@
             if (nq <= 0) continue;
             cudaStream_t cs = c == 0 ? s : chunks->stream[c - 1];
             if (c > 0) cudaStreamWaitEvent(cs, chunks->fork, 0);
+            ac.group_min = group_on ? group_min : 0;
+            ac.group_left = beside ? a.group_left + ac.q_begin / 32 + c : nullptr;
             const int np = (nq + PREP_THREADS - 1) / PREP_THREADS;
             if (a.collect_stats) { if (a.color_icp) knn_prep_kernel<true, true><<<np, PREP_THREADS, 0, cs>>>(ac); else knn_prep_kernel<false, true><<<np, PREP_THREADS, 0, cs>>>(ac); }
             else { if (a.color_icp) knn_prep_kernel<true, false><<<np, PREP_THREADS, 0, cs>>>(ac); else knn_prep_kernel<false, false><<<np, PREP_THREADS, 0, cs>>>(ac); }
             ++launches;
             if (after_prep) cudaEventRecord(after_prep, s);
-            const int group_min = getenv("ICP_GPU_GROUP_MIN") ? atoi(getenv("ICP_GPU_GROUP_MIN")) : (a.max_d2 >= 1.0f ? 8 : 0);
-            if (group_min > 0 && a.fast_path && a.use_seed && !a.color_icp) {
-                ac.group_min = group_min;
-                const int ng = (nq + GROUP_SIZE * GROUP_WARPS - 1) / (GROUP_SIZE * GROUP_WARPS);
-                if (a.collect_stats) knn_group_kernel<true><<<ng, GROUP_WARPS * 32, 0, cs>>>(ac); else knn_group_kernel<false><<<ng, GROUP_WARPS * 32, 0, cs>>>(ac);
-                ++launches;
-            }
             int nb = (nq + BVH_WARPS - 1) / BVH_WARPS;
             const int cap = std::max(1, mult * n_sms * 4 / BVH_WARPS);
             if (nb > cap) nb = cap;
-            if (a.collect_stats) { if (a.color_icp) knn_bvh_kernel<true, true><<<nb, BVH_WARPS * 32, 0, cs>>>(ac); else knn_bvh_kernel<false, true><<<nb, BVH_WARPS * 32, 0, cs>>>(ac); }
-            else { if (a.color_icp) knn_bvh_kernel<true, false><<<nb, BVH_WARPS * 32, 0, cs>>>(ac); else knn_bvh_kernel<false, false><<<nb, BVH_WARPS * 32, 0, cs>>>(ac); }
+            cudaStream_t gs = cs;
+            if (group_on) {
+                if (beside) { gs = chunks->group_stream[c]; cudaEventRecord(chunks->group_fork[c], cs); cudaStreamWaitEvent(gs, chunks->group_fork[c], 0); }
+                const int ng = (nq + GROUP_SIZE * GROUP_WARPS - 1) / (GROUP_SIZE * GROUP_WARPS);
+                if (a.collect_stats) knn_group_kernel<true><<<ng, GROUP_WARPS * 32, 0, gs>>>(ac); else knn_group_kernel<false><<<ng, GROUP_WARPS * 32, 0, gs>>>(ac);
+                ++launches;
+                if (beside) {
+                    launch_walk<WALK_LEFT>(ac, std::min(cap, n_sms * WALK_MIN_BLOCKS), gs);
+                    ++launches;
+                }
+            }
+            if (beside) launch_walk<WALK_UNOWNED>(ac, nb, cs); else launch_walk<WALK_ALL>(ac, nb, cs);
             ++launches;
+            if (beside) { cudaEventRecord(chunks->group_done[c], gs); cudaStreamWaitEvent(cs, chunks->group_done[c], 0); }
             if (c > 0) { cudaEventRecord(chunks->done[c - 1], cs); cudaStreamWaitEvent(s, chunks->done[c - 1], 0); }
         }
         if (!a.skip_finish) { match_finish_kernel<<<(a.n_src + 255) / 256, 256, 0, s>>>(a); ++launches; }
diff --git a/icp_variants_b200/csrc/registration.cu b/icp_variants_b200/csrc/registration.cu
--- a/icp_variants_b200/csrc/registration.cu
+++ b/icp_variants_b200/csrc/registration.cu
@@ -142,6 +142,7 @@
     a.weight_max_d2 = c->cfg.weight_max_distance_sq > 0.f ? c->cfg.weight_max_distance_sq : c->cfg.max_distance_sq;
     a.match_pos = (int*)c->match_pos.p; a.match_w = (float*)c->match_w.p; a.match_idx = want_idx ? (int*)c->match_idx.p : nullptr;
     a.nn_pos = (int*)c->nn_pos.p; a.qbuf = (float4*)c->qbuf.p; a.seedbuf = (float4*)c->seedbuf.p;
+    a.group_mask = (unsigned int*)c->group_mask.p; a.group_left = (int*)c->group_left.p;
     a.desc_index = desc_index;
     a.q_begin = 0; a.q_end = c->n_src;
     a.use_seed = algo == 0 ? 1 : 0;
@@ -191,6 +192,11 @@
     return 0;
 }
 
+static int group_beside() {
+    const char* e = getenv("ICP_GPU_GROUP_BESIDE");
+    return (e && atoi(e) != 0) ? 1 : 0;
+}
+
 static int enqueue_iterations(icp_gpu_ctx* ctx, const Plan& plan, int algo, std::vector<cudaEvent_t>* ev_marks) {
     MatchArgs ma; ReduceArgs ra;
     fill_match_args(ctx, ma, algo, -1, false);
@@ -201,6 +207,7 @@
     MatchChunks mc = ctx->chunks;
     mc.n = ctx->n_src >= 131072 ? 2 : 1;
     if (const char* e = getenv("ICP_GPU_MATCH_CHUNKS")) { const int v = atoi(e); if (v >= 1 && v <= ICP_MAX_MATCH_CHUNKS) mc.n = v; }
+    mc.group_beside = group_beside();
     for (int i = 0; i < plan.n_iters; ++i) {
         if (ev_marks) CU(cudaEventRecord((*ev_marks)[2 * i], ctx->stream));
         CU(icp_launch_match(ma, algo, ctx->n_sms, ctx->stream, &launches, (ev_marks && algo == 0) ? (*ev_marks)[2 * plan.n_iters + 1 + i] : nullptr, &mc));
@@ -265,6 +272,7 @@
         key.push_back((long long)(uintptr_t)ctx->mask.p); key.push_back((long long)(uintptr_t)ctx->stream);
         key.push_back(plan.n_iters);
         key.push_back(ctx->peer_world); key.push_back(ctx->peer_rank); key.push_back((long long)ctx->peer_epoch);
+        key.push_back(group_beside());
         if (!ctx->graph_exec || key != ctx->graph_key) {
             cudaGraph_t g = nullptr;
             CU(cudaStreamBeginCapture(ctx->stream, cudaStreamCaptureModeThreadLocal));
diff --git a/profiles/measure_group_beside.py b/profiles/measure_group_beside.py
--- /dev/null
+++ b/profiles/measure_group_beside.py
@@ -0,0 +1,73 @@
+import json
+import os
+import sys
+
+import numpy as np
+import torch
+
+sys.path.insert(0, os.path.dirname(os.path.dirname(os.path.abspath(__file__))))
+import bench
+from icp_variants_b200 import capi
+
+ROUNDS = int(os.environ.get("ROUNDS", "5"))
+REPS = int(os.environ.get("REPS", "7"))
+PAIRS = (("bench_pair", 0, 344, 1077), ("pair28", 28, 344, 1077), ("pair34", 34, 344, 1077), ("pair_3m", 0, 1720, 1744))
+
+
+def one_round(src, tgt, beside):
+    os.environ["ICP_GPU_GROUP_BESIDE"] = str(beside)
+    ctx = capi.Context(0)
+    try:
+        cfg = capi.default_config()
+        cfg.metric, cfg.minimizer, cfg.matching, cfg.n_iterations, cfg.max_distance_sq, cfg.nn_algorithm, cfg.collect_stats = 1, 0, 0, 30, 10.0, 2, 0
+        ctx.set_config(cfg)
+        ctx.set_target(tgt.points, tgt.normals, tgt.colors)
+        ctx.set_source(src.points, src.normals, src.colors)
+        pose, _, _ = ctx.estimate_pose(want_history=False)
+        ms = []
+        for _ in range(REPS):
+            torch.cuda.synchronize()
+            e0, e1 = torch.cuda.Event(enable_timing=True), torch.cuda.Event(enable_timing=True)
+            e0.record()
+            p, _, _ = ctx.estimate_pose(want_history=False)
+            e1.record()
+            e1.synchronize()
+            ms.append(e0.elapsed_time(e1))
+            assert np.array_equal(p, pose)
+        return float(np.median(ms)), pose
+    finally:
+        ctx.close()
+
+
+def main():
+    torch.cuda.set_device(0)
+    props = torch.cuda.get_device_properties(0)
+    out = {"what": __doc__.split("\n")[0], "device": props.name, "rounds": ROUNDS, "replays_per_round": REPS, "pairs": {}}
+    gen = capi.Context(0)
+    for name, k, sweeps, beams in PAIRS:
+        src, tgt = bench.make_pair_device_normals(gen, k, sweeps, beams)
+        ms = {0: [], 1: []}
+        poses = []
+        for r in range(ROUNDS):
+            for beside in ((0, 1) if r % 2 == 0 else (1, 0)):
+                t, pose = one_round(src, tgt, beside)
+                ms[beside].append(t)
+                poses.append(pose)
+        same = all(np.array_equal(p, poses[0]) for p in poses)
+        res = {"n_points": int(len(src)), "poses_identical": bool(same)}
+        for beside, label in ((0, "serial"), (1, "beside")):
+            v = np.array(ms[beside])
+            res[label] = {"ms_median": round(float(np.median(v)), 4), "ms_min": round(float(v.min()), 4), "ms_max": round(float(v.max()), 4),
+                          "ms_rounds": [round(float(x), 4) for x in v]}
+        res["beside_over_serial"] = round(res["beside"]["ms_median"] / res["serial"]["ms_median"], 4)
+        out["pairs"][name] = res
+        print(name, json.dumps(res), file=sys.stderr)
+    gen.close()
+    os.environ.pop("ICP_GPU_GROUP_BESIDE", None)
+    print(json.dumps(out, indent=1))
+    if not all(p["poses_identical"] for p in out["pairs"].values()):
+        sys.exit("poses differ between the schedules")
+
+
+if __name__ == "__main__":
+    main()
diff --git a/profiles/probe_timeline.py b/profiles/probe_timeline.py
--- a/profiles/probe_timeline.py
+++ b/profiles/probe_timeline.py
@@ -39,15 +39,16 @@
             torch.cuda.synchronize()
         ctx.estimate_pose(want_history=False)
         torch.cuda.synchronize()
-    tl = np.zeros((2, 2, TL_WARPS, 2), np.uint64)
+    tl = np.zeros((4, 2, TL_WARPS, 2), np.uint64)
     tr = np.zeros((512, 2), np.uint64)
     lib.icp_gpu_debug_timeline(tl.ctypes.data_as(C.c_void_p), 0)
     lib.icp_gpu_debug_timeline_reduce(tr.ctypes.data_as(C.c_void_p), 0)
     tl = tl.astype(np.int64); tr = tr.astype(np.int64)
     t0 = tl[0][tl[0][:, :, 0] > 0][:, 0].min()
-    out = {"chunks": os.environ.get("ICP_GPU_MATCH_CHUNKS", "default"), "unit": "microseconds from the iteration's first prep warp", "kernels": {}}
+    out = {"chunks": os.environ.get("ICP_GPU_MATCH_CHUNKS", "default"), "group_beside": os.environ.get("ICP_GPU_GROUP_BESIDE", "default"),
+           "device": torch.cuda.get_device_name(0), "unit": "microseconds from the iteration's first prep warp", "kernels": {}}
     spans = {}
-    for k, name in ((0, "prep"), (1, "walk")):
+    for k, name in ((0, "prep"), (1, "walk"), (2, "group"), (3, "leftover")):
         for c in range(2):
             w = tl[k, c]; w = w[w[:, 0] > 0]
             if len(w) == 0:
```

Result: no change. 219.9 (median of 6 runs) (+0.2%).
